# Helkafen/find-tfbs

Hardware: AMD Instinct MI355X
Metric: haplotype-windows scored/sec (higher is better)
Workload: dtype fp4xfp6->f32 bound + int32 exact

## Files before the change

find-tfbs_amd/__init__.py:

```python
import contextlib
import ctypes as C
from collections import namedtuple

from . import _capi
from ._capi import TfbsError, check, lib, tfbs_pattern_desc

TFBS_OK = 0
TFBS_E_NODEVICE = -10
KIND_PWM, KIND_OTHER, KIND_DIPWM = 0, 1, 2
DIR_P, DIR_N = 0, 1
NUCLEOTIDES = "ACGTN"

HIT_DTYPE = [("region", "<u4"), ("haplotype", "<u4"), ("pattern", "<u4"), ("window", "<u4"), ("start", "<u8"),
             ("end", "<u8"), ("score", "<i4"), ("reserved", "<u4")]
HITS_MODES = {"all": 0, "diff": 1}
HITS_HEADER = "#chrom\tregion\thaplotype\tcarriers\tkind\tname\tpattern_id\tstrand\tstart\tend\tscore\tcarrier_ids\n"
BEST_DTYPE = [("region", "<u4"), ("haplotype", "<u4"), ("pattern", "<u4"), ("range", "<u4"), ("window", "<u4"),
              ("n_windows", "<u4"), ("score", "<i4"), ("reserved", "<u4"), ("start", "<u8"), ("end", "<u8")]
BEST_MODES = {"all": 0, "diff": 1}
BEST_HEADER = ("#chrom\tregion\tbed\tinner_start\tinner_end\tname\tpattern_id\thaplotype\tcarriers\tkind\tstrand\t"
               "start\tend\tscore\tdelta\tcarrier_ids\n")
AFFINITY_DTYPE = [("region", "<u4"), ("haplotype", "<u4"), ("pattern", "<u4"), ("range", "<u4"), ("n_windows", "<u4"),
                  ("n_nonzero", "<u4"), ("sum", "<u8")]
AFFINITY_MODES = {"all": 0, "diff": 1}
# ... 254 lines not shown
    return [NUCLEOTIDES.index(n.nuc if isinstance(n, NucleotidePos) else n[0]) for n in hap]


def patch_haplotype(rng, diffs, ref_haplotype):
    L = lib()
    nd = len(diffs)
    dref = [NUCLEOTIDES.index(c) for d in diffs for c in d.reference]
    dalt = [NUCLEOTIDES.index(c) for d in diffs for c in d.alternative]
    n = len(ref_haplotype)
    cap = n + sum(len(d.alternative) for d in diffs) + 8
    on = (C.c_uint8 * cap)()
    op = (C.c_uint64 * cap)()
    nout = C.c_size_t()
    check(L.tfbs_patch_haplotype(
        rng[0], rng[1], nd, (C.c_uint64 * max(1, nd))(*[d.pos for d in diffs]),
        (C.c_uint8 * max(1, len(dref)))(*dref), (C.c_uint32 * max(1, nd))(*[len(d.reference) for d in diffs]),
        (C.c_uint8 * max(1, len(dalt)))(*dalt), (C.c_uint32 * max(1, nd))(*[len(d.alternative) for d in diffs]),
        (C.c_uint8 * max(1, n))(*_nuc_codes(ref_haplotype)),
        (C.c_uint64 * max(1, n))(*[x[1] for x in ref_haplotype]), n, on, op, cap, C.byref(nout)))
    return [NucleotidePos(NUCLEOTIDES[on[i]], op[i]) for i in range(nout.value)]


def counts_as_genotypes(v1, v2, verbose=False):
    n = len(v1)
    maf = C.c_uint32()
    info = C.create_string_buffer(64 + 16 * n)
    gts = C.create_string_buffer(64 + 24 * n)
    r = check(lib().tfbs_counts_as_genotypes((C.c_uint32 * max(1, n))(*v1), (C.c_uint32 * max(1, n))(*v2), n,
                                             C.byref(maf), info, len(info), gts, len(gts)))
    if r != 1:
        return None
    s = info.value.decode()
    counts_part, freqs_part = s.split(";")
    counts = [int(x) for x in counts_part[len("COUNTS="):].split(",")]
    f0, f1, f2 = (int(x) for x in freqs_part[len("freqs="):].split("/"))
    return counts, maf.value, f0, f1, f2, gts.value.decode()


def scores_as_genotypes(left, right, min_spread=1):
    n = len(left)
    maf = C.c_uint32()
    info = C.create_string_buffer(128)
    gts = C.create_string_buffer(16 + 11 * n)
    r = check(lib().tfbs_scores_as_genotypes((C.c_int32 * max(1, n))(*left), (C.c_int32 * max(1, n))(*right), n,
                                             min_spread, C.byref(maf), info, len(info), gts, len(gts)))
    if r != 1:
        return None
    return maf.value, info.value.decode(), gts.value.decode()


PATH_BITS = {"FAST": 1 << 0, "BIG": 1 << 1, "WALK": 1 << 2, "STEPBITS": 1 << 3, "DIRTY_LISTED": 1 << 4,
             "COR_ARENA": 1 << 5, "LISTS_SLICED": 1 << 6, "RUNS_L2": 1 << 7, "HAP_GLOBAL": 1 << 8, "U32": 1 << 9,
             "CNT_ARENA": 1 << 10, "TICKET": 1 << 11, "GIVEUP": 1 << 12, "ASM": 1 << 16, "ASM_HAPS": 1 << 17,
             "ASM_RUNS": 1 << 18, "ASM_HITS": 1 << 19, "ASM_REFS": 1 << 20, "ASM_SCRATCH": 1 << 21}
PATH_WHY_SHIFT = 13


def path_why(word):
    return (word >> PATH_WHY_SHIFT) & 7


class Scanner:

    def __init__(self, patterns, device=0):
        self.patterns = patterns if isinstance(patterns, PatternSet) else PatternSet.from_patterns(patterns)
        self.h = C.c_void_p()
        check(lib().tfbs_ctx_create(device, self.patterns.h, C.byref(self.h)))

    def close(self):
        if getattr(self, "h", None):
            lib().tfbs_ctx_destroy(self.h)
            self.h = None

    def __del__(self):
        self.close()

    def rows_bgzf_blocks(self):
        out = (C.c_uint64 * 3)()
        check(lib().tfbs_ctx_rows_bgzf_blocks(self.h, out))
        return dict(zip(("blocks", "wave", "stored"), (int(x) for x in out)))

    def assembly_trace(self, on=True):
        check(lib().tfbs_ctx_assembly_trace(self.h, 1 if on else 0))

    def assembly_figures(self):
        out = (C.c_uint64 * 8)()
        check(lib().tfbs_ctx_assembly_figures(self.h, out))
        return dict(zip(("left", "arena", "spill", "wide", "leftover", "reruns", "reruns_wide", "reruns_leftover"),
                        (int(x) for x in out)))

    def post_figures(self):
        out = (C.c_uint64 * 4)()
        check(lib().tfbs_ctx_post_figures(self.h, out))
        return dict(zip(("left_out", "reruns_post", "fused", "cand"), (int(x) for x in out)))

    def matches_all(self, haplotype):
        n = len(haplotype)
        nucs = (C.c_uint8 * max(1, n))(*_nuc_codes(haplotype))
        pos = (C.c_uint64 * max(1, n))(*[x[1] for x in haplotype])
        npat = len(self.patterns)
        counts = (C.c_uint32 * max(1, npat))()
        total = C.c_size_t()
        cap = 64
        while True:
            s = (C.c_uint64 * cap)()
            e = (C.c_uint64 * cap)()
            rc = lib().tfbs_matches(self.h, nucs, pos, n, counts, s, e, cap, C.byref(total))
            if rc == -1 and total.value > cap:
                cap = total.value
                continue
            check(rc)
            break
        out, k = [], 0
        for i in range(npat):
            out.append([(s[k + j], e[k + j]) for j in range(counts[i])])
            k += counts[i]
        return out

    def matches(self, pattern_index, haplotype, haplotype_ids=()):
        p = self.patterns[pattern_index]
        ids = tuple(haplotype_ids)
        return [Match(Range(a, b), p.pattern_id, ids) for a, b in self.matches_all(haplotype)[pattern_index]]

    def last_scan_ms(self):
        return lib().tfbs_ctx_last_scan_ms(self.h)

    def last_best_ms(self):
        out = (C.c_double * 2)()
        check(lib().tfbs_ctx_last_best_ms(self.h, out))
        return out[0], out[1]

    def last_affinity_ms(self):
        out = (C.c_double * 2)()
        check(lib().tfbs_ctx_last_affinity_ms(self.h, out))
        return out[0], out[1]

    def last_scores_ms(self):
        out = (C.c_double * 4)()
        check(lib().tfbs_ctx_last_scores_ms(self.h, out))
        return tuple(out)

    def last_effects_ms(self):
        out = (C.c_double * 3)()
        check(lib().tfbs_ctx_last_effects_ms(self.h, out))
        return out[0], out[1], out[2]

    def last_mutscan_ms(self):
        out = (C.c_double * 4)()
        check(lib().tfbs_ctx_last_mutscan_ms(self.h, out))
        return tuple(out)


def mutscan_ring_max_length():
    return lib().tfbs_mutscan_ring_max_length()


def mutscan_kinds_mask(kinds):
    if isinstance(kinds, int):
        return kinds
    names = kinds.split(",") if isinstance(kinds, str) else list(kinds)
    mask = 0
    for k in names:
        mask |= 1 << MUT_KINDS.index(k)
    return mask


# ... 758 lines not shown
```

find-tfbs_amd/_capi.py:

```python
import ctypes as C
import os

HERE = os.path.dirname(os.path.abspath(__file__))
LIB_PATH = os.environ.get("TFBS_LIB") or os.path.join(HERE, "lib", "libtfbs_amd.so")

u8p = C.POINTER(C.c_uint8)
u16p = C.POINTER(C.c_uint16)
u32p = C.POINTER(C.c_uint32)
u64p = C.POINTER(C.c_uint64)
i32p = C.POINTER(C.c_int32)
vp = C.c_void_p


class tfbs_pattern_desc(C.Structure):
    _fields_ = [
        ("pattern_id", C.c_uint16),
        ("direction", C.c_uint8),
        ("kind", C.c_uint8),
        ("length", C.c_uint32),
        ("weights", i32p),
        ("min_score", C.c_int32),
        ("name", C.c_char_p),
    ]

# ... 77 lines not shown
class tfbs_run_ext_affinity(C.Structure):
    _fields_ = tfbs_run_ext_mutscan._fields_ + [("affinity_output", C.c_char_p), ("affinity_mode", C.c_int)]


SIGNATURES = [
    ("tfbs_strerror", C.c_char_p, [C.c_int]),
    ("tfbs_last_error", C.c_char_p, []),
    ("tfbs_version", C.c_char_p, []),
    ("tfbs_patterns_create", C.c_int, [C.POINTER(tfbs_pattern_desc), C.c_size_t, C.POINTER(vp)]),
    ("tfbs_patterns_from_files", C.c_int, [C.c_char_p, C.c_char_p, C.c_float, C.c_char_p, C.c_int, C.POINTER(vp)]),
    ("tfbs_patterns_from_files_di", C.c_int, [C.c_char_p, C.c_char_p, C.c_char_p, C.c_float, C.c_char_p, C.c_int,
                                              C.POINTER(vp)]),
    ("tfbs_patterns_count", C.c_size_t, [vp]),
    ("tfbs_patterns_get", C.c_int, [vp, C.c_size_t, C.POINTER(tfbs_pattern_desc)]),
    ("tfbs_patterns_name_of", C.c_char_p, [vp, C.c_uint16]),
    ("tfbs_patterns_max_length", C.c_uint32, [vp]),
    ("tfbs_patterns_destroy", None, [vp]),
    ("tfbs_patterns_plan_stats", C.c_int, [vp, C.c_uint32, C.c_int, C.POINTER(tfbs_plan_stats)]),
    ("tfbs_patterns_dinuc_stats", C.c_int, [vp, u32p, u32p, u64p]),
    ("tfbs_patterns_dinuc_lut_scores", C.c_int, [vp, C.c_size_t, u8p, C.c_size_t, i32p]),
    ("tfbs_patterns_mfma_bound", C.c_int, [vp, C.c_size_t, C.POINTER(C.c_uint8), C.POINTER(tfbs_mfma_bound)]),
    ("tfbs_patterns_mfma_plan", C.c_int, [vp, C.c_uint32, u8p, C.c_size_t, C.POINTER(C.c_size_t),
                                          C.POINTER(tfbs_mfma_super), C.c_size_t, C.POINTER(C.c_size_t), i32p,
                                          C.c_size_t, C.POINTER(C.c_size_t)]),
    ("tfbs_patterns_score_tails", C.c_int, [vp, C.c_int, C.c_size_t, i32p, C.c_size_t, u64p, u64p]),
    ("tfbs_patterns_pvalue_thresholds", C.c_int, [vp, C.c_int, C.c_double, i32p]),
    ("tfbs_patterns_with_min_scores", C.c_int, [vp, i32p, C.POINTER(vp)]),
    ("tfbs_patterns_from_files_pvalue", C.c_int, [C.c_char_p, C.c_char_p, C.c_char_p, C.c_int, C.c_int, C.c_double,
                                                  C.POINTER(vp)]),
    ("tfbs_pvalue_tile_widths", None, [u32p]),
    ("tfbs_parse_weight", C.c_int, [C.c_char_p, i32p]),
    ("tfbs_parse_threshold_file", C.c_int, [C.c_char_p, C.c_float, i32p]),
    ("tfbs_device_count", C.c_int, [C.POINTER(C.c_int)]),
    ("tfbs_ctx_create", C.c_int, [C.c_int, vp, C.POINTER(vp)]),
    ("tfbs_ctx_destroy", None, [vp]),
    ("tfbs_ctx_sync", C.c_int, [vp]),
    ("tfbs_ctx_set_host_threads", C.c_int, [vp, C.c_uint32]),
    ("tfbs_ctx_last_scan_ms", C.c_float, [vp]),
    ("tfbs_ctx_last_scan_launches", C.c_int, [vp]),
    ("tfbs_ctx_last_mfma_ms", C.c_float, [vp]),
    ("tfbs_ctx_window_lists", C.c_int, [vp, C.POINTER(C.c_uint64), C.POINTER(C.c_double)]),
    ("tfbs_ctx_scan_counters", C.c_int, [vp, C.POINTER(C.c_uint64)]),
    ("tfbs_matches", C.c_int, [vp, u8p, u64p, C.c_size_t, u32p, u64p, u64p, C.c_size_t, C.POINTER(C.c_size_t)]),
    ("tfbs_patch_haplotype", C.c_int, [C.c_uint64, C.c_uint64, C.c_size_t, u64p, u8p, u32p, u8p, u32p, u8p, u64p,
                                       C.c_size_t, u8p, u64p, C.c_size_t, C.POINTER(C.c_size_t)]),
    ("tfbs_batch_create", C.c_int, [vp, C.c_uint32, C.c_int, C.POINTER(vp)]),
    ("tfbs_batch_destroy", None, [vp]),
    ("tfbs_batch_add_bed", C.c_int, [vp, C.c_char_p]),
    ("tfbs_batch_set_window_lmax", C.c_int, [vp, C.c_uint32]),
    ("tfbs_batch_set_build_device", C.c_int, [vp, C.c_int]),
    ("tfbs_batch_hold", C.c_int, [vp, C.c_int]),
    ("tfbs_batch_group_calls", C.c_int, [vp, u64p]),
    ("tfbs_batch_build_stats", C.c_int, [vp, u64p, u64p]),
    ("tfbs_grouper_create", C.c_int, [C.c_int, C.POINTER(vp)]),
    ("tfbs_grouper_destroy", None, [vp]),
    ("tfbs_grouper_group", C.c_int, [vp, C.c_uint32, C.c_size_t, u32p, u32p, u32p, u32p, u64p, u32p, C.c_size_t,
                                     C.POINTER(C.c_size_t), u16p]),
    ("tfbs_batch_patch_stats", C.c_int, [vp, u64p]),
    ("tfbs_batch_region_ext", C.c_int, [vp, C.c_uint64, C.c_uint64, u64p, u64p]),
    ("tfbs_batch_region_begin", C.c_int, [vp, C.c_uint64, C.c_uint64, C.c_char_p, C.c_size_t]),
    ("tfbs_batch_region_add_inner", C.c_int, [vp, C.c_uint32, C.c_uint64, C.c_uint64]),
    ("tfbs_batch_region_add_record_gt", C.c_int, [vp, C.c_uint64, C.c_uint32, C.c_char_p, C.c_char_p, i32p]),
    ("tfbs_batch_region_add_record_carriers", C.c_int, [vp, C.c_uint64, C.c_char_p, C.c_char_p, u32p, C.c_size_t]),
    ("tfbs_batch_region_end", C.c_int, [vp]),
    ("tfbs_batch_num_regions", C.c_size_t, [vp]),
    ("tfbs_batch_num_haplotypes", C.c_size_t, [vp]),
    ("tfbs_batch_num_windows", C.c_uint64, [vp]),
    ("tfbs_batch_num_effective_windows", C.c_uint64, [vp]),
    ("tfbs_batch_num_cell_ops", C.c_uint64, [vp]),
    ("tfbs_batch_num_scan_windows", C.c_uint64, [vp]),
    ("tfbs_batch_num_scan_cell_ops", C.c_uint64, [vp]),
    ("tfbs_batch_input_bytes", C.c_uint64, [vp]),
    ("tfbs_batch_output_bytes", C.c_uint64, [vp]),
    ("tfbs_batch_upload", C.c_int, [vp, vp]),
    ("tfbs_scan", C.c_int, [vp, vp]),
    ("tfbs_batch_download", C.c_int, [vp, vp]),
    ("tfbs_batch_reduce", C.c_int, [vp, vp]),
    ("tfbs_batch_assemble", C.c_int, [vp, vp]),
    ("tfbs_batch_assemble_wait", C.c_int, [vp, vp]),
    ("tfbs_step", C.c_int, [vp, vp]),
    ("tfbs_ctx_last_assemble_ms", C.c_float, [vp]),
    ("tfbs_ctx_assembly_trace", C.c_int, [vp, C.c_int]),
    ("tfbs_batch_assembly_paths", C.c_int, [vp, vp, u32p, C.c_uint32]),
    ("tfbs_ctx_assembly_figures", C.c_int, [vp, u64p]),
    ("tfbs_ctx_post_figures", C.c_int, [vp, u64p]),
    ("tfbs_batch_region_layout", C.c_int, [vp, C.c_size_t, u32p]),
    ("tfbs_batch_region_hap_runs", C.c_int, [vp, C.c_size_t, C.c_uint32, C.POINTER(C.c_int), u32p, u32p, u32p,
                                            C.c_uint32]),
    ("tfbs_batch_region_hap_own_runs", C.c_int, [vp, C.c_size_t, C.c_uint32, C.POINTER(C.c_int), u32p, u32p, u32p,
                                                C.c_uint32]),
    ("tfbs_batch_encode",C.c_int, [vp, vp, C.c_size_t, C.c_size_t]),
    ("tfbs_batch_encode_flags", C.c_int, [vp, vp, C.c_size_t, C.c_size_t, C.c_int]),
    ("tfbs_batch_encode_stats", C.c_int, [vp, u64p]),
    ("tfbs_ctx_rows_bgzf_seconds", C.c_int, [vp, C.POINTER(C.c_double)]),
    ("tfbs_ctx_rows_bgzf_blocks", C.c_int, [vp, u64p]),
    ("tfbs_batch_rows_bgzf", C.c_int, [vp, vp, C.c_size_t, C.c_size_t, C.c_char_p, C.c_uint32, u32p, C.c_int,
                                       u64p, u64p, u64p]),
    ("tfbs_batch_region_num_keys", C.c_int, [vp, C.c_size_t, C.POINTER(C.c_size_t)]),
    ("tfbs_batch_region_key", C.c_int, [vp, C.c_size_t, C.c_size_t, u32p, u64p, u64p, u16p, u32p, u32p]),
    ("tfbs_batch_rows", C.c_int, [vp, C.c_char_p, C.c_uint32, u32p, C.POINTER(C.c_void_p), C.POINTER(C.c_size_t)]),
    ("tfbs_batch_region_rows", C.c_int, [vp, C.c_size_t, C.c_char_p, C.c_uint32, u32p, C.POINTER(C.c_void_p),
                                         C.POINTER(C.c_size_t)]),
    ("tfbs_batch_region_digest", C.c_int, [vp, C.c_size_t, u64p]),
    ("tfbs_batch_region_key_digest_sum", C.c_int, [vp, C.c_size_t, u64p]),
    ("tfbs_batch_region_input_digest", C.c_int, [vp, C.c_size_t, u64p]),
    ("tfbs_batch_region_digests", C.c_int, [vp, C.c_size_t, C.c_size_t, C.c_uint32, C.c_uint32, u64p, u64p, u64p]),
    ("tfbs_batch_region_stats", C.c_int, [vp, C.c_size_t, u32p, u32p]),
    ("tfbs_batch_format_rows", C.c_int, [vp, C.c_char_p, C.c_uint32, C.c_uint32, C.c_size_t, C.c_size_t, u64p,
                                         u64p]),
    ("tfbs_batch_prep_seconds", C.c_int, [vp, C.POINTER(C.c_double)]),
    ("tfbs_batch_hits", C.c_int, [vp, vp, C.c_size_t, C.c_size_t, C.POINTER(C.c_void_p), C.POINTER(C.c_size_t)]),
    ("tfbs_batch_hits_count", C.c_int, [vp, vp, C.c_size_t, C.c_size_t, u64p]),
    ("tfbs_ctx_last_hits_ms", C.c_int, [vp, C.POINTER(C.c_double)]),
    ("tfbs_batch_region_haplotype", C.c_int, [vp, C.c_size_t, C.c_uint32, u8p, u64p, C.c_size_t,
                                              C.POINTER(C.c_size_t), u32p]),
    ("tfbs_batch_region_membership", C.c_int, [vp, C.c_size_t, u32p]),
    ("tfbs_batch_hits_tsv", C.c_int, [vp, C.c_void_p, C.c_size_t, C.c_char_p, C.c_int, C.POINTER(C.c_void_p),
                                      C.POINTER(C.c_size_t)]),
    ("tfbs_batch_best", C.c_int, [vp, vp, C.c_size_t, C.c_size_t, C.POINTER(C.c_void_p), C.POINTER(C.c_size_t)]),
    ("tfbs_batch_region_num_ranges", C.c_int, [vp, C.c_size_t, C.POINTER(C.c_size_t)]),
    ("tfbs_batch_region_range", C.c_int, [vp, C.c_size_t, C.c_size_t, u64p, u64p]),
    ("tfbs_ctx_last_best_ms", C.c_int, [vp, C.POINTER(C.c_double)]),
    ("tfbs_batch_best_tsv", C.c_int, [vp, C.c_void_p, C.c_size_t, C.c_char_p, C.c_int, C.POINTER(C.c_void_p),
                                      C.POINTER(C.c_size_t)]),
    ("tfbs_affinity_weight", C.c_uint64, [C.c_uint64]),
    ("tfbs_patterns_affinity_tops", C.c_int, [vp, i32p]),
    ("tfbs_batch_affinity", C.c_int, [vp, vp, C.c_size_t, C.c_size_t, C.POINTER(C.c_void_p), C.POINTER(C.c_size_t)]),
    ("tfbs_ctx_last_affinity_ms", C.c_int, [vp, C.POINTER(C.c_double)]),
    ("tfbs_batch_affinity_tsv", C.c_int, [vp, C.c_void_p, C.c_size_t, C.c_char_p, C.c_int, C.POINTER(C.c_void_p),
                                          C.POINTER(C.c_size_t)]),
    ("tfbs_batch_keep_variants", C.c_int, [vp, C.c_int]),
    ("tfbs_batch_region_variant", C.c_int, [vp, C.c_size_t, C.c_size_t, u64p, u8p, u8p, C.c_size_t,
                                            C.POINTER(C.c_size_t), C.POINTER(C.c_size_t), u32p, u32p, u32p]),
    ("tfbs_batch_effects", C.c_int, [vp, vp, C.c_size_t, C.c_size_t, C.POINTER(C.c_void_p), C.POINTER(C.c_size_t)]),
    ("tfbs_ctx_last_effects_ms", C.c_int, [vp, C.POINTER(C.c_double)]),
    ("tfbs_batch_effects_tsv", C.c_int, [vp, C.c_void_p, C.c_size_t, C.c_char_p, C.c_int, C.POINTER(C.c_void_p),
                                         C.POINTER(C.c_size_t)]),
    ("tfbs_batch_mutscan", C.c_int, [vp, vp, C.c_size_t, C.c_size_t, C.c_uint32, C.POINTER(C.c_void_p),
                                     C.POINTER(C.c_size_t)]),
    ("tfbs_batch_mutscan_count", C.c_int, [vp, vp, C.c_size_t, C.c_size_t, C.c_uint32, u64p]),
    ("tfbs_mutscan_ring_max_length", C.c_uint32, []),
    ("tfbs_ctx_last_mutscan_ms", C.c_int, [vp, C.POINTER(C.c_double)]),
    ("tfbs_batch_mutscan_tsv", C.c_int, [vp, C.c_void_p, C.c_size_t, C.c_char_p, C.POINTER(C.c_void_p),
                                         C.POINTER(C.c_size_t)]),
    ("tfbs_scores_as_genotypes", C.c_int, [i32p, i32p, C.c_size_t, C.c_uint64, u32p, C.c_char_p, C.c_size_t,
                                           C.c_char_p, C.c_size_t]),
    ("tfbs_batch_score_rows", C.c_int, [vp, vp, C.c_size_t, C.c_size_t, C.c_char_p, C.c_uint32, C.c_uint64, u32p,
                                        C.POINTER(C.c_void_p), C.POINTER(C.c_size_t), u64p]),
    ("tfbs_ctx_last_scores_ms", C.c_int, [vp, C.POINTER(C.c_double)]),
    ("tfbs_free", None, [C.c_void_p]),
    ("tfbs_counts_as_genotypes", C.c_int, [u32p, u32p, C.c_size_t, u32p, C.c_char_p, C.c_size_t, C.c_char_p,
                                           C.c_size_t]),
    ("tfbs_run", C.c_int, [C.c_void_p]),
    ("tfbs_run_ex", C.c_int, [C.c_void_p, C.c_void_p]),
    ("tfbs_bcf_open", C.c_int, [C.c_char_p, C.POINTER(vp)]),
    ("tfbs_inflate_raw", C.c_int, [C.c_void_p, C.c_size_t, C.c_void_p, C.c_size_t]),
    ("tfbs_bcf_close", None, [vp]),
    ("tfbs_bcf_select", C.c_int, [vp, C.POINTER(C.c_size_t), C.c_size_t]),
    ("tfbs_bcf_num_samples", C.c_size_t, [vp]),
    ("tfbs_bcf_indexed", C.c_int, [vp]),
    ("tfbs_bcf_sample_name", C.c_char_p, [vp, C.c_size_t]),
    ("tfbs_bcf_fetch", C.c_int, [vp, C.c_char_p, C.c_uint64, C.c_uint64, C.POINTER(C.c_size_t)]),
    ("tfbs_bcf_set_carriers_mode", C.c_int, [vp, C.c_int]),
    ("tfbs_bcf_record_carriers", C.c_int, [vp, C.c_size_t, C.POINTER(u32p), C.POINTER(C.c_size_t), C.POINTER(C.c_int)]),
    ("tfbs_bcf_record", C.c_int, [vp, C.c_size_t, u64p, u32p, u32p, C.POINTER(C.c_char_p), C.POINTER(C.c_char_p),
                                  C.POINTER(i32p)]),
# ... 47 lines not shown
```

find-tfbs_amd/csrc/ctx.hpp:

```cpp
#pragma once

#include <hip/hip_runtime.h>

#include <algorithm>
#include <atomic>
#include <cerrno>
#include <chrono>
#include <condition_variable>
#include <cstdint>
#include <cstdio>
#include <cstdlib>
#include <cstring>
#include <deque>
#include <functional>
#include <memory>
#include <mutex>
#include <string>
#include <thread>
#include <vector>

#include "batch.hpp"
#include "bgzf_gpu.hpp"
#include "hip_util.hpp"
#include "hits.hpp"
#include "keys.hpp"
#include "patterns.hpp"
#include "rows.hpp"
#include "scan.hpp"
#include "scores.hpp"
#include "tfbs_internal.hpp"

namespace tfbs {

int env_int(const char *name, int dflt);

struct PlanTables {
    DevBuf<DevUnit> fast_units;
    DevBuf<DevPattern> gen_pats;
    DevBuf<DevTile> fast_tiles, gen_tiles;
    DevBuf<int32_t> lut, wfull, gen_w, m_image, m_weights, m_meta;
    DevBuf<DevUnit> di_units;
    DevBuf<DevTile> di_tiles;
    DevBuf<int32_t> di_lut, di_w;
    DevBuf<uint8_t> slot_mfma;
    DevBuf<DevMSuper> m_supers;
    template <class F>
    void each_buf(F &&f) const {
        f(fast_units), f(gen_pats), f(fast_tiles), f(gen_tiles), f(lut), f(wfull), f(gen_w), f(m_image);
        f(m_weights), f(m_meta), f(di_units), f(di_tiles), f(di_lut), f(di_w), f(slot_mfma), f(m_supers);
    }
};

struct Knobs {
    uint32_t tile_blocks = (uint32_t)std::min(36, std::max(8, env_int("TFBS_TILE_BLOCKS", 20)));
    uint32_t haps_per_block = (uint32_t)std::max(8, env_int("TFBS_HAPS_PER_BLOCK", 128));
    bool mfma = env_int("TFBS_MFMA", 1) != 0;
    uint32_t mfma_lds = (uint32_t)std::min(144, std::max(8, env_int("TFBS_MFMA_LDS_KB", 44))) * 1024u;
    uint32_t mfma_hpb = (uint32_t)std::min((int)kMMaxHapsPerBlock, std::max(4, env_int("TFBS_MFMA_HAPS_PER_BLOCK", 64)));
    uint32_t cand_cap = (uint32_t)std::min(1 << 16, std::max(64, env_int("TFBS_CAND_CAP", 1024)));
    uint32_t scan_unit_env = [](int u) { return u == 1 || u == 2 || u == 4 ? u : 0; }(env_int("TFBS_SCAN_UNIT", 0));
    uint32_t scan_unit_words_env = [](const char *uw) {
        return uw && !strcmp(uw, "lds") ? 1u : uw && !strcmp(uw, "global") ? 2u : 0u;
    }(getenv("TFBS_SCAN_UNIT_WORDS"));
    bool debug_over = env_int("TFBS_DEBUG_OVER", 0) != 0;
    bool kf_prof_on = env_int("TFBS_KF_PROF", 0) != 0;
    bool kf_persistent = env_int("TFBS_KF_PERSIST", 1) != 0;
    uint32_t kf_grid = (uint32_t)std::max(0, env_int("TFBS_KF_GRID", 0));
    int kf_big_u = env_int("TFBS_KF_BIGU", (int)key_fast_big_u());
    uint32_t key_fast_max_u = (uint32_t)std::max(0, env_int("TFBS_KEY_FAST_MAXU", 1 << 30));
    uint32_t key_cor_lds = (uint32_t)std::max(0, env_int("TFBS_KEY_COR_LDS", 1 << 30));
    int asm_lean_mode = env_int("TFBS_ASM_LEAN", 1);
    bool post_fuse_env = env_int("TFBS_POST_FUSE", 0) != 0;
    bool step_graphs = env_int("TFBS_STEP_GRAPH", 1) != 0 && !getenv("TFBS_SCAN_PROF") && !kf_prof_on && !debug_over;
};

struct BatchImage {
    DevBuf<uint32_t> words, nmask, counts;
    bool counts_live = false;
    DevBuf<int32_t> posrel, inner;
    DevBuf<DevHap> haps;
    DevBuf<uint32_t> druns;
    DevBuf<DevRegion> regions;
    uint32_t n_regions = 0;
    const tfbs_batch *resident = nullptr;
    uint64_t upload_gen = 0;
    uint32_t mfma_group_words = 0;
    template <class F>
    void each_buf(F &&f) const {
        f(words), f(nmask), f(counts), f(posrel), f(inner), f(haps), f(druns), f(regions);
    }
};

struct WindowLists {
    DevBuf<uint64_t> wl_off[2], wl_tmp;
    DevBuf<uint32_t> wl[2];
    DevBuf<uint16_t> wl16[2];
    DevBuf<uint8_t> gnarrow;
    DevBuf<uint32_t> gorder;
    DevBuf<uint32_t> gcost;
    bool wl_any_narrow = false, wl_any_wide = false;
    DevBuf<uint4> hd, hd2;
    uint64_t wl_entries[2] = {0, 0};
    double wl_seconds = 0;
    uint32_t wl_n_haps = 0;
    uint32_t scan_unit = 1;
    bool wl_share = false;
    DevBuf<uint64_t> sh_off[2], sh_stat;
    DevBuf<uint2> sh[2];
    DevBuf<uint32_t> sh_cur;
    DevBuf<ClassTab> sh_tab;
    uint64_t sh_entries[2] = {0, 0};
    uint64_t sh_listed[2][2] = {{0, 0}, {0, 0}};
    template <class F>
    void each_buf(F &&f) const {
        f(gnarrow), f(gorder), f(hd), f(hd2);
        for (int c = 0; c < 2; c++) f(wl_off[c]), f(wl[c]), f(wl16[c]), f(sh_off[c]), f(sh[c]);
    }
};

struct ScanState {
    Event ev0, ev1;
    Event evk0, evk1;
    Event over_ev;
    bool kernel_timed = false;
    float last_kernel_ms = 0.f, last_ms = 0.f;
    int last_launches = 0;
    bool timing_pending = false;
    bool scanned = false;
    DevBuf<uint32_t> cands;
    DevBuf<uint32_t> hitl, hitn;
    DevBuf<uint32_t> candn;
    DevBuf<uint32_t> ref_hits, ref_count;
    DevBuf<uint32_t> spill, over;
    uint32_t spill_cap = 1u << 16;
    DevBuf<uint32_t> spill_sorted, spill_bcnt, spill_boff;
    bool spill_cnt_ctr = false;
    DevBuf<uint32_t> cand_over;
    uint32_t cand_over_cap = 1u << 20;
    DevBuf<unsigned long long> hits;
    PinnedArray<uint32_t> over_host;
    bool over_pending = false;
    bool over_copied = false;
    bool post_done = false;
    ScanArgs last_margs{};
    uint32_t scan_cand_cap = 1024;
    uint32_t scan_hit_cap = 1024;
    bool post_fuse_ok = false, post_fused = false;
    DevBuf<unsigned long long> scan_prof;
    template <class F>
    void each_buf(F &&f) const {
        f(cands), f(hitl), f(hitn), f(candn), f(ref_hits), f(ref_count), f(spill), f(over), f(spill_sorted);
        f(spill_bcnt), f(spill_boff), f(cand_over), f(hits);
    }
};

struct AsmStages {
    bool wide = true, leftover = true, post = true, post_fused = false;
};

struct AsmState {
    Stream side;
    Event kf_fork, kf_join;
    Event asm_ev, asm_t0, asm_t1;
    DevBuf<uint32_t> asm_scratch;
    DevBuf<uint32_t> key_first, var_counts, asm_redo;
    DevBuf<uint32_t> asm_ctr;
    DevBuf<uint32_t> cor_arena;
    uint32_t cor_cap = 1u << 22;
    DevBuf<uint8_t> key_flags;
    DevBuf<DevVarKey> var_keys;
    uint32_t var_keys_cap = 1u << 16;
    uint64_t var_cap = 1u << 24;
// ... 156 lines not shown
```

find-tfbs_amd/csrc/ctx_assembly.hip:

```cpp
#include "ctx.hpp"

using namespace tfbs;

AsmArgs tfbs::asm_args(tfbs_ctx *ctx, const Batch &B, int mode) {
    AsmArgs a{};
    a.haps = ctx->img.haps.p;
    a.druns = ctx->img.druns.p;
    a.regions = ctx->img.regions.p;
    a.inner = ctx->img.inner.p;
    a.mmeta = ctx->tabs.m_meta.p;
    a.slot_mfma = ctx->tabs.slot_mfma.p;
    a.any_dense = (!ctx->plan.fast_tiles.empty() || !ctx->plan.gen_tiles.empty() || !ctx->plan.di_tiles.empty()) ? 1 : 0;
    a.n_slots = B.n_slots;
    a.hpb = ctx->knobs.mfma_hpb;
    a.hitl = ctx->scan.hitl.p;
    a.hitn = ctx->scan.hitn.p;
    a.cand_cap = ctx->scan.scan_hit_cap;
    a.mfma = ctx->plan.m_supers.empty() ? 0 : 1;
    a.ref_hits = ctx->scan.ref_hits.p;
    a.ref_count = ctx->scan.ref_count.p;
    a.spill_sorted = ctx->scan.spill_sorted.p;
    a.spill_off = ctx->scan.spill_boff.p;
    a.spill_cnt = ctx->scan.spill_cnt_ctr ? ctx->asmb.asm_ctr.p + kAsmCtrWords : ctx->scan.spill_bcnt.p;
    a.spill_count = ctx->plan.m_supers.empty() ? nullptr : ctx->scan.over.p;
    a.spill_cap = ctx->scan.spill_cap;
    a.counts = ctx->img.counts_live ? ctx->img.counts.p : nullptr;
    a.dense_base = ctx->img.counts_live ? 1 : 0;
    a.scratch = ctx->asmb.asm_scratch.p;
    a.mode = mode;
    return a;
}

static int enqueue_assembly(tfbs_ctx *ctx, Batch &B, bool post) {
    int rc;
    const uint64_t n_keys = (uint64_t)(B.inner.size() / 2) * B.n_slots;
    const uint32_t nr = (uint32_t)B.regions.size();
    if ((rc = ctx->asmb.key_first.ensure(std::max<uint64_t>(n_keys, 1))) ||
        (rc = ctx->asmb.key_flags.ensure(std::max<uint64_t>(n_keys, 1))) || (rc = ctx->asmb.asm_ctr.ensure(kAsmCtrWords + asm_bucket_words(nr))) ||
        (rc = ctx->asmb.asm_redo.ensure((size_t)nr + 1)) || (rc = ctx->asmb.cor_arena.ensure(ctx->asmb.cor_cap)))
        return rc;
    if (!ctx->asmb.asm_host) HIP_TRY(ctx->asmb.asm_host.alloc(kAsmCtrWords));
    if (const int vc = env_int("TFBS_VAR_CAP", 0); vc > 0) {
        if (!ctx->asmb.var_cap_forced) {
            ctx->asmb.var_keys_cap = (uint32_t)vc;
            ctx->asmb.var_cap = 4ull * (uint32_t)vc;
            ctx->asmb.var_cap_forced = true;
        }
    } else {
        ctx->asmb.var_keys_cap = std::max<uint32_t>(ctx->asmb.var_keys_cap, (uint32_t)std::min<uint64_t>(n_keys / 16, 1u << 26));
        ctx->asmb.var_cap = std::max<uint64_t>(ctx->asmb.var_cap, std::min<uint64_t>(B.n_counts / 16, 1ull << 28));
    }
    if ((rc = ctx->asmb.var_keys.ensure(ctx->asmb.var_keys_cap)) || (rc = ctx->asmb.var_counts.ensure(ctx->asmb.var_cap))) return rc;
    if (!ctx->step.capturing) HIP_TRY(hipEventRecord(ctx->asmb.asm_t0, ctx->stream));
    const bool mfma = !ctx->plan.m_supers.empty();
    if (!(mfma && post && ctx->asmb.asm_ctr_zeroed && ctx->img.n_regions == nr))
        HIP_TRY(hipMemsetAsync(ctx->asmb.asm_ctr.p, 0, (kAsmCtrWords + (mfma && post ? asm_bucket_words(nr) : 0)) * 4,
                               ctx->stream));
    ctx->asmb.asm_ctr_zeroed = false;
    const bool lean = mfma && post && !ctx->asmb.asm_full && ctx->knobs.asm_lean_mode != 0;
    ctx->asmb.stages.wide = !(lean && (ctx->knobs.asm_lean_mode == 2 || ctx->asmb.prev_spill <= kPostSerial));
    ctx->asmb.stages.leftover = !(lean && (ctx->knobs.asm_lean_mode == 2 || ctx->asmb.prev_redo == 0));
    if (mfma && post) {
        ctx->asmb.stages.post = true;
        ctx->asmb.stages.post_fused = ctx->scan.post_fused;
        if (ctx->scan.post_fused) {
            ctx->asmb.stages.wide = false;
        } else if (asm_skips_post(ctx)) {
            ctx->asmb.stages.post = ctx->asmb.stages.wide = false;
        } else if ((rc = launch_post_fused(ctx->scan.last_margs, !ctx->scan.post_done, ctx->asmb.asm_ctr.p + kCtrWgDone,
                                           std::max<uint32_t>(1, nr), ctx->asmb.asm_ctr.p + kAsmCtrWords, ctx->scan.spill_boff.p,
                                           ctx->scan.spill_sorted.p, ctx->stream, ctx->asmb.stages.wide, ctx->asmb.asm_ctr.p,
                                           ctx->asmb.asm_ctr.p + kCtrNeedWide, lean && ctx->asmb.prev_cand == 0 ? 1u : 256u))) {
            return rc;
        }
        if (ctx->asmb.stages.post) {
            ctx->scan.post_done = true;
            ctx->scan.spill_cnt_ctr = true;
        }
    }
    ctx->scan.post_fused = false;
    AsmArgs a = asm_args(ctx, B, 0);
    if (mfma && !ctx->asmb.stages.post) a.spill_count = nullptr;
    a.report_fast = mfma && !ctx->asmb.stages.post ? 1u : 0u;
    a.key_first = ctx->asmb.key_first.p;
    a.key_flags = ctx->asmb.key_flags.p;
    a.var_keys = ctx->asmb.var_keys.p;
    a.var_keys_cap = ctx->asmb.var_keys_cap;
    a.var_counts = ctx->asmb.var_counts.p;
    a.var_cap = ctx->asmb.var_cap;
    a.var_tot = reinterpret_cast<unsigned long long *>(ctx->asmb.asm_ctr.p + kCtrVarTot);
    a.redo = ctx->asmb.asm_redo.p;
    a.redo_n = ctx->asmb.asm_ctr.p + kCtrRedoN;
    a.fast_max_u = ctx->knobs.key_fast_max_u;
    a.cor_arena = ctx->asmb.cor_arena.p;
    a.cor_cap = ctx->asmb.cor_cap;
    a.cor_used = ctx->asmb.asm_ctr.p + kCtrCorUsed;
    a.cor_lds = ctx->knobs.key_cor_lds;
    a.why = ctx->knobs.debug_over ? ctx->asmb.asm_ctr.p + kCtrWhy : nullptr;
    a.report_src = mfma ? ctx->scan.over.p : nullptr;
    a.report = ctx->asmb.asm_ctr.p;
    a.order = ctx->asmb.asm_order_n == nr ? ctx->asmb.asm_order.p : nullptr;
    a.persist = ctx->knobs.kf_persistent ? 1u : 0u;
    a.next = ctx->asmb.asm_ctr.p + kCtrNext;
    a.grid_cap = ctx->knobs.kf_grid;
    ctx->asmb.asm_traced = ctx->asmb.asm_trace;
    if (ctx->asmb.asm_trace && nr) {
        if ((rc = ctx->asmb.asm_path.ensure(nr))) return rc;
        HIP_TRY(hipMemsetAsync(ctx->asmb.asm_path.p, 0, (size_t)nr * 4, ctx->stream));
        a.path = ctx->asmb.asm_path.p;
    }
    if (ctx->knobs.kf_prof_on && nr) {
        if ((rc = ctx->asmb.kf_prof.ensure((size_t)nr * 16))) return rc;
        HIP_TRY(hipMemsetAsync(ctx->asmb.kf_prof.p, 0, (size_t)nr * 128, ctx->stream));
        a.prof = ctx->asmb.kf_prof.p;
    }
    if ((rc = launch_key_fast(a, nr, a.order ? ctx->asmb.asm_order_big : 0, ctx->stream, ctx->asmb.side, ctx->asmb.kf_fork,
                              ctx->asmb.kf_join, ctx->asmb.stages.leftover)) ||
        (nr == 0 && (rc = launch_asm_report(a.report_src, ctx->asmb.asm_ctr.p, ctx->stream))))
        return rc;
    if (!ctx->step.capturing) HIP_TRY(hipEventRecord(ctx->asmb.asm_t1, ctx->stream));
    HIP_TRY(hipMemcpyAsync(ctx->asmb.asm_host.p, ctx->asmb.asm_ctr.p, 4 * kAsmCtrWords, hipMemcpyDeviceToHost, ctx->stream));
    if (!ctx->step.capturing) HIP_TRY(hipEventRecord(ctx->asmb.asm_ev, ctx->stream));
    ctx->scan.over_pending = false;
    ctx->asmb.asm_batch = &B;
    ctx->asmb.asm_state = 1;
    ctx->asmb.asm_timed = true;
    return TFBS_OK;
}

static int kf_prof_report(tfbs_ctx *ctx, uint32_t nr) {
    std::vector<uint64_t> h((size_t)nr * 16);
    HIP_TRY(hipMemcpy(h.data(), ctx->asmb.kf_prof.p, h.size() * 8, hipMemcpyDeviceToHost));
    double ph[6] = {0, 0, 0, 0, 0, 0}, sz[8] = {0, 0, 0, 0, 0, 0, 0, 0}, mx = 0, at = 0;
    uint32_t n = 0;
    for (uint32_t r = 0; r < nr; r++) {
        const uint64_t *p = &h[(size_t)r * 16];
        if (!p[6]) continue;
        n++;
        for (int k = 0; k < 6; k++) ph[k] += (double)(p[k + 1] - p[k]);
        mx = std::max(mx, (double)(p[6] - p[0]));
        at += (double)p[7];
        for (int k = 0; k < 8; k++) sz[k] += (double)p[8 + k];
    }
    std::vector<std::pair<double, uint32_t>> tot;
    for (uint32_t r = 0; r < nr; r++)
        if (h[(size_t)r * 16 + 6]) tot.push_back({(double)(h[(size_t)r * 16 + 6] - h[(size_t)r * 16]), r});
    std::sort(tot.begin(), tot.end());
    if (!tot.empty()) {
        auto pct = [&](double f) { return tot[std::min(tot.size() - 1, (size_t)(f * tot.size()))].first; };
        fprintf(stderr, "[kf prof] total ticks p50 %.0f p90 %.0f p99 %.0f max %.0f; slowest regions (ticks U rows chunks "
                        "corrections refs):", pct(0.5), pct(0.9), pct(0.99), tot.back().first);
        for (size_t i = tot.size(); i-- > 0 && i + 6 > tot.size();) {
            const uint64_t *p = &h[(size_t)tot[i].second * 16];
            fprintf(stderr, " [%.0f %llu %llu %llu %llu %llu]", tot[i].first, (unsigned long long)p[8],
                    (unsigned long long)p[12], (unsigned long long)p[13], (unsigned long long)p[11],
                    (unsigned long long)p[15]);
        }
        fprintf(stderr, "\n");
    }
    uint64_t t_lo = UINT64_MAX, t_hi = 0;
    double busy = 0;
    for (uint32_t r = 0; r < nr; r++) {
        const uint64_t *p = &h[(size_t)r * 16];
        if (!p[6]) continue;
        t_lo = std::min(t_lo, p[0]);
        t_hi = std::max(t_hi, p[6]);
        busy += (double)(p[6] - p[0]);
    }
    {
        std::vector<std::pair<std::pair<uint64_t, uint64_t>, uint32_t>> ev;
        for (uint32_t r = 0; r < nr; r++)
            if (h[(size_t)r * 16 + 6]) ev.push_back({{h[(size_t)r * 16 + 14], h[(size_t)r * 16]}, r});
        std::sort(ev.begin(), ev.end());
        double gap = 0, late = 0, early_end = 0;
        uint32_t n_gap = 0, n_groups = 0;
        for (size_t i = 0; i < ev.size(); i++) {
            const uint64_t *p = &h[(size_t)ev[i].second * 16];
            const bool first = i == 0 || ev[i - 1].first.first != ev[i].first.first;
            const bool last = i + 1 == ev.size() || ev[i + 1].first.first != ev[i].first.first;
            if (first) {
                n_groups++;
                late += (double)(p[0] - t_lo);
            } else {
                gap += (double)(p[0] - h[(size_t)ev[i - 1].second * 16 + 6]);
                n_gap++;
            }
            if (last) early_end += (double)(t_hi - p[6]);
        }
        if (n_groups)
            fprintf(stderr, "[kf prof] %u workgroups: mean gap between a workgroup's regions %.1f us (%u gaps), first "
                            "region start after the kernel's first %.1f us, last end before the kernel's last %.1f us\n",
                    n_groups, n_gap ? gap / n_gap / 100.0 : 0.0, n_gap, late / n_groups / 100.0, early_end / n_groups / 100.0);
    }
    uint32_t early = 0;
    for (uint32_t r = 0; r < nr; r++)
        if (h[(size_t)r * 16 + 6] && h[(size_t)r * 16] < t_lo + 1000) early++;
    if (t_hi > t_lo)
        fprintf(stderr, "[kf prof] span %.1f us (first region start to last end, 100 MHz ticks), region-time %.1f us: "
                        "%.0f regions in flight on average; %u regions started in the first 10 us\n",
                (t_hi - t_lo) / 100.0, busy / 100.0, busy / (double)(t_hi - t_lo), early);
    const double d = n ? n : 1;
    fprintf(stderr,
            "[kf prof] regions %u of %u ticks/region: descr+hitn %.0f refs %.0f dirty %.0f lists %.0f keys %.0f "
            "chunks %.0f (of which var-list atomics %.0f) (max total %.0f); per region: U %.1f entries %.1f dirty-refs %.1f corrections %.1f rows "
            "%.1f chunks %.2f in-LDS %.2f refs %.1f\n",
            n, nr, ph[0] / d, ph[1] / d, ph[2] / d, ph[3] / d, ph[4] / d, ph[5] / d, at / d, mx, sz[0] / d, sz[1] / d,
            sz[2] / d, sz[3] / d, sz[4] / d, sz[5] / d, sz[6] / d, sz[7] / d);
    return TFBS_OK;
}

int tfbs::assembly_wait(tfbs_ctx *ctx, Batch &B) {
    for (int round = 0; ctx->asmb.asm_state == 1; round++) {
        if (round == 8) return tfbs::fail(TFBS_E_NOMEM, "scan / key lists still full after 8 reruns");
        HIP_TRY(hipEventSynchronize(ctx->asmb.asm_ev));
        const uint32_t nspill = ctx->asmb.asm_host[kCtrOver], ncand = ctx->asmb.asm_host[kCtrOver + 1];
        const uint64_t *vt = reinterpret_cast<const uint64_t *>(ctx->asmb.asm_host.p + kCtrVarTot);
        const uint64_t nk = vt[0], nc = vt[1];
        if (ctx->knobs.debug_over && ctx->asmb.asm_host[kCtrRedoN]) {
            std::vector<uint32_t> redo(ctx->asmb.asm_host[kCtrRedoN]);
            HIP_TRY(hipMemcpy(redo.data(), ctx->asmb.asm_redo.p, redo.size() * 4, hipMemcpyDeviceToHost));
            uint64_t su = 0, sr = 0;
            uint32_t mu = 0, mi = 0;
            for (uint32_t r : redo) {
                const DevRegion &rg = B.regions[r];
                su += rg.hap_count;
                mu = std::max(mu, rg.hap_count);
                mi = std::max(mi, rg.n_inner);
                for (uint32_t l = 0; l < rg.hap_count; l++) sr += B.haps[rg.hap_begin + l].n_druns;
            }
            const uint32_t *why = ctx->asmb.asm_host.p + kCtrWhy;
            fprintf(stderr, "tfbs assembly: %zu regions left to key_asm: mean haplotypes %.1f (max %u), max inner %u, "
                            "mean diff runs %.1f; reasons: shape %u lists %u runs %u refs %u arena(cor) %u arena(cnt) %u\n",
                    redo.size(), (double)su / redo.size(), mu, mi, (double)sr / redo.size(), why[0], why[1], why[2],
                    why[3], why[4], why[5]);
        }
        if (ctx->knobs.debug_over)
            fprintf(stderr, "tfbs assembly: spill %u/%u candidates %u/%u left to key_asm %u arena %u/%u varying keys "
                            "%llu/%u counts %llu/%llu\n", nspill, ctx->scan.spill_cap, ncand, ctx->scan.cand_over_cap,
                    ctx->asmb.asm_host[kCtrRedoN], ctx->asmb.asm_host[kCtrCorUsed], ctx->asmb.cor_cap,
                    (unsigned long long)nk, ctx->asmb.var_keys_cap, (unsigned long long)nc,
                    (unsigned long long)ctx->asmb.var_cap);
        int rc;
        const bool need_post = !ctx->asmb.stages.post && (nspill || ncand);
        const bool need_wide = !ctx->asmb.stages.wide && ctx->asmb.asm_host[kCtrNeedWide], need_left = !ctx->asmb.stages.leftover && ctx->asmb.asm_host[kCtrRedoN];
        if (need_post || need_wide || need_left) {
            ctx->asmb.asm_full = true;
            ctx->asmb.asm_reruns++;
            ctx->asmb.asm_reruns_post += need_post ? 1 : 0;
            ctx->asmb.asm_post_rerun = need_post;
            ctx->asmb.asm_reruns_wide += need_wide ? 1 : 0;
            ctx->asmb.asm_reruns_left += need_left ? 1 : 0;
            rc = enqueue_assembly(ctx, B, true);
            ctx->asmb.asm_full = false;
            if (rc) return rc;
            continue;
        }
        if (ctx->asmb.asm_host[kCtrCorUsed] > ctx->asmb.cor_cap)
            ctx->asmb.cor_cap = (uint32_t)std::min<uint64_t>((uint64_t)ctx->asmb.asm_host[kCtrCorUsed] * 5 / 4, 1u << 30);
        if (nspill > ctx->scan.spill_cap || ncand > ctx->scan.cand_over_cap) {
            grow_cap(ctx->scan.spill_cap, ncand > ctx->scan.cand_over_cap ? 2 * std::max(nspill, 1024u) : nspill, UINT32_MAX / 4);
            grow_cap(ctx->scan.cand_over_cap, ncand, UINT32_MAX / 4);
            const int n = launch_scan(ctx, (uint32_t)B.haps.size(), nullptr, 0);
            if (n < 0) return n;
            if ((rc = enqueue_assembly(ctx, B, true))) return rc;
            continue;
        }
        if (nk > ctx->asmb.var_keys_cap || nc > ctx->asmb.var_cap) {
            if (nk >= (1ull << 32) || nc >= (1ull << 40)) return tfbs::fail(TFBS_E_NOMEM, "too many varying counts");
            ctx->asmb.var_keys_cap = (uint32_t)std::max<uint64_t>(ctx->asmb.var_keys_cap, std::min<uint64_t>(nk + nk / 4 + 1024, UINT32_MAX));
            ctx->asmb.var_cap = std::max<uint64_t>(ctx->asmb.var_cap, nc + nc / 4 + 4096);
            if ((rc = enqueue_assembly(ctx, B, false))) return rc;
            continue;
        }
        ctx->asmb.asm_state = 2;
        ctx->asmb.asm_reruns_wide += ctx->asmb.asm_post_rerun && nspill > kPostSerial ? 1 : 0;
        ctx->asmb.asm_post_rerun = false;
        ctx->asmb.prev_spill = nspill;
        ctx->asmb.prev_redo = ctx->asmb.asm_host[kCtrRedoN];
        ctx->asmb.prev_cand = ncand;
        if (ctx->knobs.kf_prof_on && (rc = kf_prof_report(ctx, (uint32_t)B.regions.size()))) return rc;
    }
    return TFBS_OK;
}

// ... 276 lines not shown
```

find-tfbs_amd/csrc/ctx_scan.hip:

```cpp
#include "ctx.hpp"

using namespace tfbs;

__global__ void zero3_kernel(uint32_t *__restrict__ a, uint32_t na, uint32_t *__restrict__ b, uint32_t nb,
                             uint32_t *__restrict__ c, uint32_t nc) {
    const uint32_t s = gridDim.x * blockDim.x;
    for (uint32_t k = blockIdx.x * blockDim.x + threadIdx.x; k < na || k < nb || k < nc; k += s) {
        if (k < na) a[k] = 0;
        if (k < nb) b[k] = 0;
        if (k < nc) c[k] = 0;
    }
}

constexpr uint32_t kUnitPairs = 2 * kMBlockWaves;
static uint32_t scan_unit_for(const tfbs_ctx *ctx, uint32_t n_groups) {
    if (ctx->knobs.scan_unit_env) return ctx->knobs.scan_unit_env;
    for (int c = 0; c < 2; c++)
        if (ctx->lists.wl_entries[c] > (uint64_t)kUnitPairs * 64 * n_groups) return 1;
    for (uint32_t G = kMMaxUnit; G > 1; G /= 2)
        if (2 * (uint64_t)((n_groups + G - 1) / G) >= 3 * (uint64_t)(2 * ctx->n_cus)) return G;
    return 1;
}

int tfbs::build_lists(tfbs_ctx *ctx, uint32_t n_haps, const std::vector<uint8_t> &narrow, Batch *B) {
    const Plan &P = ctx->plan;
    ctx->lists.wl_share = false;
    ctx->lists.wl_n_haps = n_haps;
    for (int c = 0; c < 2; c++) ctx->lists.sh_entries[c] = ctx->lists.sh_listed[c][0] = ctx->lists.sh_listed[c][1] = 0;
    if (B) B->lists_counted = false;
    if (P.m_supers.empty()) return TFBS_OK;
    const auto t0 = std::chrono::steady_clock::now();
    uint32_t lmin[2] = {0, 0}, span[2] = {0, 0};
    for (const DevMSuper &S : P.m_supers) {
        uint32_t &l = lmin[S.nk > 2 ? 1 : 0];
        l = l ? std::min(l, S.lmin) : S.lmin;
        span[S.nk > 2 ? 1 : 0] = std::max(span[S.nk > 2 ? 1 : 0], S.lmax);
    }
    int rc;
    for (int c = 0; c < 2; c++)
        if (lmin[c] && (rc = ctx->lists.wl_off[c].ensure((size_t)n_haps + 1))) return rc;
    if ((rc = ctx->lists.wl_tmp.ensure(scan_tmp_words((size_t)n_haps + 1))) ||
        (rc = ctx->img.druns.ensure(std::max<size_t>(ctx->img.druns.n, 1))))
        return rc;
    if ((rc = ctx->lists.gnarrow.put(narrow, ctx->stream))) return rc;
    WindowListBufs bufs{};
    for (int c = 0; c < 2; c++) {
        bufs.off[c] = lmin[c] ? ctx->lists.wl_off[c].p : nullptr;
        bufs.list[c] = nullptr;
        bufs.list16[c] = nullptr;
    }
    bufs.gnarrow = narrow.empty() ? nullptr : ctx->lists.gnarrow.p;
    if ((rc = ctx->lists.hd.ensure(std::max<uint32_t>(n_haps, 1))) || (rc = ctx->lists.hd2.ensure(std::max<uint32_t>(n_haps, 1))))
        return rc;
    bufs.hd = ctx->lists.hd.p;
    bufs.hd2 = ctx->lists.hd2.p;
    bufs.scan_tmp = ctx->lists.wl_tmp.p;
    ctx->lists.wl_any_narrow = ctx->lists.wl_any_wide = false;
    for (uint8_t g : narrow) (g ? ctx->lists.wl_any_narrow : ctx->lists.wl_any_wide) = true;
    if (narrow.empty()) ctx->lists.wl_any_wide = true;
    auto ensure = [](void *x, int c, uint64_t n, uint32_t **p, uint16_t **p16) {
        tfbs_ctx *cx = static_cast<tfbs_ctx *>(x);
        if (int e = cx->lists.wl[c].ensure(cx->lists.wl_any_wide ? n : 1)) return e;
        if (int e = cx->lists.wl16[c].ensure(cx->lists.wl_any_narrow ? n : 1)) return e;
        *p = cx->lists.wl[c].p;
        *p16 = cx->lists.wl16[c].p;
        return TFBS_OK;
    };
    const bool share = B && B->dedup && n_haps && env_int("TFBS_SHARE", 1) != 0;
    std::vector<std::pair<uint32_t, uint32_t>> rest;
    if (share) {
        std::vector<ClassTab> tab(2, ClassTab{});
        rest = B->pwm_len_hist;
        for (size_t t = 0; t * kGMetaInts < P.m_meta.size(); t++) {
            const int32_t *gm = &P.m_meta[t * kGMetaInts];
            ClassTab &ct = tab[gm[kGDepth] > 2];
            for (int sn = 0; sn < kMStrands; sn++) {
                if (gm[kGOrig + sn] < 0) continue;
                const uint32_t L = (uint32_t)gm[kGStrandInts * sn + kGLen];
                for (uint32_t r = L; r <= 32; r++) ct.w[r] += 1, ct.c[r] += L;
                for (auto &lc : rest)
                    if (lc.first == L && lc.second) lc.second--;
            }
        }
        if ((rc = ctx->lists.sh_tab.put(tab, ctx->stream)) || (rc = ctx->lists.sh_stat.ensure(4)) ||
            (rc = ctx->lists.sh_cur.ensure(2 * (size_t)n_haps)))
            return rc;
        for (int c = 0; c < 2; c++)
            if (lmin[c] && (rc = ctx->lists.sh_off[c].ensure((size_t)n_haps + 1))) return rc;
        HIP_TRY(hipStreamSynchronize(ctx->stream));
        for (int c = 0; c < 2; c++) bufs.soff[c] = lmin[c] ? ctx->lists.sh_off[c].p : nullptr;
        bufs.scur = ctx->lists.sh_cur.p;
        bufs.stat = ctx->lists.sh_stat.p;
    }
    auto ensure_share = [](void *x, int c, uint64_t n, uint2 **p) {
        tfbs_ctx *cx = static_cast<tfbs_ctx *>(x);
        if (int e = cx->lists.sh[c].ensure(n)) return e;
        *p = cx->lists.sh[c].p;
        return TFBS_OK;
    };
    if ((rc = build_window_lists(ctx->img.haps.p, n_haps, ctx->img.druns.p, lmin, span, ctx->knobs.mfma_hpb, 1, bufs, ctx->lists.wl_entries,
                                 ctx->stream, ensure, ctx, share ? 1u : 0u, ctx->img.regions.p, ctx->img.words.p, ctx->lists.sh_tab.p,
                                 ensure_share, ctx->lists.sh_entries, ctx->lists.sh_listed)))
        return rc;
    ctx->lists.wl_share = share;
    if (share) {
        B->list_windows = ctx->lists.sh_listed[0][0] + ctx->lists.sh_listed[1][0];
        B->list_cell_ops = ctx->lists.sh_listed[0][1] + ctx->lists.sh_listed[1][1];
        for (const auto &lc : rest) {
            if (!lc.second) continue;
            uint64_t nw = 0;
            for (const DevHap &h : B->haps) nw += h.len >= lc.first ? h.len - lc.first + 1 : 0;
            B->list_windows += nw * lc.second;
            B->list_cell_ops += nw * lc.second * lc.first;
        }
        B->lists_counted = true;
    }
    for (int c = 0; c < 2; c++)
        if (!lmin[c]) ctx->lists.wl_off[c].release(), ctx->lists.wl[c].release(), ctx->lists.wl16[c].release();
    ctx->lists.gorder.release();
    ctx->lists.scan_unit = scan_unit_for(ctx, (n_haps + ctx->knobs.mfma_hpb - 1) / ctx->knobs.mfma_hpb);
    if (env_int("TFBS_SCAN_LPT", 1) && n_haps) {
// ... 196 lines not shown
            HIP_TRY(hipEventRecord(ctx->scan.over_ev, ctx->stream));
            ctx->scan.over_copied = true;
        }
        HIP_TRY(hipEventSynchronize(ctx->scan.over_ev));
        uint32_t nspill = ctx->scan.over_host[0];
        const uint32_t ncand = ctx->scan.over_host[1];
        if (ncand > 0 && ncand <= ctx->scan.cand_over_cap && !ctx->scan.post_done) {
            const int f = launch_post_scan(ctx->scan.last_margs, ctx->stream);
            if (f < 0) return f;
            HIP_TRY(hipMemcpyAsync(ctx->scan.over_host.p, ctx->scan.over.p, 8, hipMemcpyDeviceToHost, ctx->stream));
            HIP_TRY(hipStreamSynchronize(ctx->stream));
            nspill = ctx->scan.over_host[0];
        }
        if (ctx->knobs.debug_over) {
            fprintf(stderr, "tfbs_scan overflow lists: spill %u/%u candidates %u/%u\n", nspill, ctx->scan.spill_cap, ncand,
                    ctx->scan.cand_over_cap);
            const size_t nw = ctx->scan.hitn.n;
            std::vector<uint32_t> hn(nw);
            HIP_TRY(hipMemcpy(hn.data(), ctx->scan.hitn.p, nw * 4, hipMemcpyDeviceToHost));
            uint64_t sh = 0, mh = 0;
            for (size_t i = 0; i < nw; i++) sh += hn[i], mh = std::max<uint64_t>(mh, hn[i]);
            fprintf(stderr, "tfbs_scan hit pairs %llu (max per wave %llu) over %zu waves\n", (unsigned long long)sh,
                    (unsigned long long)mh, nw);
        }
        if (nspill <= ctx->scan.spill_cap && ncand <= ctx->scan.cand_over_cap) {
            ctx->scan.over_pending = false;
            ctx->scan.post_done = true;
            if (nspill) {
                const uint32_t nr = std::max<uint32_t>(1, ctx->img.n_regions);
                const int rc = launch_spill_buckets(ctx->scan.over.p, ctx->scan.spill_cap, ctx->scan.spill.p, nr, ctx->scan.spill_bcnt.p,
                                                    ctx->scan.spill_boff.p, ctx->scan.spill_sorted.p, ctx->stream);
                if (rc) return rc;
                ctx->scan.spill_cnt_ctr = false;
            }
            return TFBS_OK;
        }
        grow_cap(ctx->scan.spill_cap, ncand > ctx->scan.cand_over_cap ? 2 * std::max(nspill, 1024u) : nspill, UINT32_MAX / 4);
        grow_cap(ctx->scan.cand_over_cap, ncand, UINT32_MAX / 4);
        const int n = launch_scan(ctx, n_haps, hits, wpp);
        if (n < 0) return n;
    }
    return TFBS_OK;
}

extern "C" {

int tfbs_ctx_group_pairs(tfbs_ctx *ctx, int cls, uint32_t *pairs, size_t cap, size_t *n_groups) {
    if (!ctx || !n_groups || cls < 0 || cls > 1 || (cap && !pairs)) return tfbs::fail(TFBS_E_ARG, "bad argument");
    const uint32_t n = ctx->lists.wl_n_haps, hpb = ctx->knobs.mfma_hpb;
    *n_groups = ((size_t)n + hpb - 1) / hpb;
    if (*n_groups > cap) return cap ? tfbs::fail(TFBS_E_ARG, "group pairs: the array is too small") : TFBS_OK;
    if (!ctx->lists.wl_off[cls].p) {
        for (size_t g = 0; g < *n_groups; g++) pairs[g] = 0;
        return TFBS_OK;
    }
    HIP_TRY(hipSetDevice(ctx->device));
    std::vector<uint64_t> off((size_t)n + 1);
    HIP_TRY(hipStreamSynchronize(ctx->stream));
    HIP_TRY(hipMemcpy(off.data(), ctx->lists.wl_off[cls].p, off.size() * 8, hipMemcpyDeviceToHost));
    for (size_t g = 0; g < *n_groups; g++) {
        const uint64_t nw = off[std::min<size_t>((g + 1) * hpb, n)] - off[g * hpb];
        pairs[g] = (uint32_t)(((nw + 31) / 32 + 1) / 2);
    }
    return TFBS_OK;
}

int tfbs_ctx_share_entries(tfbs_ctx *ctx, int cls, uint32_t *entries, size_t cap, size_t *n_haps) {
    if (!ctx || !n_haps || cls < 0 || cls > 1 || (cap && !entries)) return tfbs::fail(TFBS_E_ARG, "bad argument");
    const uint32_t n = ctx->lists.wl_n_haps;
    *n_haps = n;
    if (n > cap) return cap ? tfbs::fail(TFBS_E_ARG, "share entries: the array is too small") : TFBS_OK;
    if (!ctx->lists.wl_share || !ctx->lists.wl_off[cls].p || !ctx->lists.sh_entries[cls]) {
        for (size_t h = 0; h < n; h++) entries[h] = 0;
        return TFBS_OK;
    }
    HIP_TRY(hipSetDevice(ctx->device));
    std::vector<uint64_t> off((size_t)n + 1);
    HIP_TRY(hipStreamSynchronize(ctx->stream));
    HIP_TRY(hipMemcpy(off.data(), ctx->lists.sh_off[cls].p, off.size() * 8, hipMemcpyDeviceToHost));
    for (size_t h = 0; h < n; h++) entries[h] = (uint32_t)(off[h + 1] - off[h]);
    return TFBS_OK;
}

int tfbs_batch_upload(tfbs_ctx *ctx, tfbs_batch *b) {
    if (!ctx || !b) return tfbs::fail(TFBS_E_ARG, "null argument");
    Batch &B = b->b;
    if (B.pats != ctx->pats) return tfbs::fail(TFBS_E_ARG, "batch and ctx use different pattern sets");
    if (B.open) return tfbs::fail(TFBS_E_STATE, "region still open");
    if (B.slot_pid != ctx->plan.slot_pid) return tfbs::fail(TFBS_E_STATE, "batch slot order differs from the ctx plan");
    HIP_TRY(hipSetDevice(ctx->device));
    uint64_t big = 0;
    for (DevRegion &rg : B.regions) {
        rg.big_off = big;
        if (rg.hap_count > key_asm_lds_counters()) big += rg.hap_count;
    }
    const bool dense = !ctx->plan.fast_tiles.empty() || !ctx->plan.gen_tiles.empty() || !ctx->plan.di_tiles.empty();
    int rc;
    if ((rc = ctx->img.words.put(B.words, ctx->stream)) || (rc = ctx->img.nmask.put(B.nmask, ctx->stream)) ||
        (rc = ctx->img.posrel.put(B.posrel, ctx->stream)) || (rc = ctx->img.haps.put(B.haps, ctx->stream)) ||
        (rc = ctx->img.druns.put(B.druns, ctx->stream)) ||
        (rc = ctx->img.regions.put(B.regions, ctx->stream)) || (rc = ctx->img.inner.put(B.inner, ctx->stream)) ||
        (rc = ctx->asmb.asm_scratch.ensure(std::max<uint64_t>(big, 1))) ||
        (dense && (rc = ctx->img.counts.ensure(std::max<uint64_t>(B.n_counts, 1)))))
        return rc;
    std::vector<uint32_t> order(B.regions.size());
    {
        for (uint32_t i = 0; i < order.size(); i++) order[i] = i;
        std::stable_sort(order.begin(), order.end(), [&](uint32_t x, uint32_t y) {
            return B.regions[x].hap_count > B.regions[y].hap_count;
        });
        if ((rc = ctx->asmb.asm_order.put(order, ctx->stream))) return rc;
        ctx->asmb.asm_order_n = (uint32_t)order.size();
        ctx->asmb.asm_order_big = 0;
        const int big_u = ctx->knobs.kf_big_u;
        while (big_u > 0 && ctx->asmb.asm_order_big < order.size() &&
               B.regions[order[ctx->asmb.asm_order_big]].hap_count > (uint32_t)big_u)
            ctx->asmb.asm_order_big++;
    }
    std::vector<uint8_t> narrow((B.haps.size() + ctx->knobs.mfma_hpb - 1) / ctx->knobs.mfma_hpb, 1);
    for (size_t h = 0; h < B.haps.size(); h++)
        if (B.haps[h].len > kWlNarrowLen) narrow[h / ctx->knobs.mfma_hpb] = 0;
    if ((rc = build_lists(ctx, (uint32_t)B.haps.size(), narrow, &B))) return rc;
    HIP_TRY(hipStreamSynchronize(ctx->stream));
    ctx->img.counts_live = dense;
    ctx->img.resident = b;
    ctx->img.upload_gen++;
    ctx->asmb.prev_spill = ctx->asmb.prev_redo = ctx->asmb.prev_cand = UINT32_MAX;
    ctx->img.mfma_group_words = mfma_group_words(B.haps.data(), (uint32_t)B.haps.size(), ctx->knobs.mfma_hpb);
    ctx->img.n_regions = (uint32_t)B.regions.size();
    ctx->scan.over_pending = false;
    ctx->scan.scanned = false;
    ctx->asmb.asm_state = 0;
    return TFBS_OK;
}

int tfbs_scan(tfbs_ctx *ctx, tfbs_batch *b) {
    if (!ctx || !b) return tfbs::fail(TFBS_E_ARG, "null argument");
    if (ctx->img.resident != b) return tfbs::fail(TFBS_E_STATE, "batch not uploaded to this ctx");
    HIP_TRY(hipSetDevice(ctx->device));
    if (!ctx->step.capturing) HIP_TRY(hipEventRecord(ctx->scan.ev0, ctx->stream));
    ctx->scan.kernel_timed = false;
    const int n = launch_scan(ctx, (uint32_t)b->b.haps.size(), nullptr, 0);
    if (n < 0) return n;
    ctx->scan.scanned = true;
    ctx->asmb.asm_state = 0;
    if (!ctx->step.capturing) HIP_TRY(hipEventRecord(ctx->scan.ev1, ctx->stream));
    ctx->scan.last_launches = n;
    ctx->scan.timing_pending = true;
    b->b.counts_valid = b->b.reduced = false;
    b->b.enc_r0 = b->b.enc_r1 = 0;
    return TFBS_OK;
}

int tfbs_batch_download(tfbs_ctx *ctx, tfbs_batch *b) {
    if (!ctx || !b) return tfbs::fail(TFBS_E_ARG, "null argument");
    if (ctx->img.resident != b) return tfbs::fail(TFBS_E_STATE, "batch not resident on this ctx");
    if (!ctx->scan.scanned) return tfbs::fail(TFBS_E_STATE, "batch not scanned (tfbs_scan)");
    HIP_TRY(hipSetDevice(ctx->device));
    Batch &B = b->b;
    int rc;
    if (ctx->asmb.asm_state == 1 && ctx->asmb.asm_batch == &B && (rc = assembly_wait(ctx, B))) return rc;
    if ((rc = check_overflow(ctx, (uint32_t)B.haps.size()))) return rc;
    if (!ctx->img.counts_live) {
        if ((rc = ctx->img.counts.ensure(std::max<uint64_t>(B.n_counts, 1)))) return rc;
    }
    AsmArgs a = asm_args(ctx, B, 1);
// ... 90 lines not shown
```

find-tfbs_amd/csrc/key_kernels.hip:

```cpp
#include <hip/hip_runtime.h>

#include <mutex>

#include <algorithm>
#include <cstdio>
#include <cstdlib>
#include <string>
#include <type_traits>

#include "keys.hpp"

namespace tfbs {
namespace {

constexpr int kAsmBlock = 256;
constexpr uint32_t kAsmWaves = kAsmBlock / 64;
constexpr uint32_t kAsmCounters = 6144;
constexpr uint32_t kAsmHaps = 1024;

constexpr uint32_t kAsmRuns = 2048;
constexpr uint32_t kAsmHits = 2048;
constexpr uint32_t kAsmRefs = 256;
constexpr uint32_t kAsmKeyWords = 2048;
constexpr uint32_t kAsmKeyWin = 32 * kAsmKeyWords;

__device__ __forceinline__ uint2 spill_range(const AsmArgs &A, uint32_t r) {
    if (!A.spill_count || !*A.spill_count) return make_uint2(0, 0);
    const uint32_t c = A.spill_cnt[r];
    if (c == 0) return make_uint2(0, 0);
    const uint32_t o = A.spill_off[r];
    return make_uint2(o, o + c);
}

__device__ __forceinline__ uint32_t ref_overlaps(const AsmArgs &A, const DevRegion &rg, uint32_t L, uint32_t i,
                                                 uint32_t k0, uint32_t nk) {
    const int32_t *inner = A.inner + 2 * (size_t)rg.inner_off;
    uint32_t mask = 0;
    for (uint32_t k = k0; k < k0 + nk; k++) {
        const int32_t s = inner[2 * k], en = inner[2 * k + 1];
        const uint32_t span = (uint32_t)(en - s);
        if ((uint32_t)((int32_t)i - s) <= span || (uint32_t)((int32_t)(i + L) - 1 - s) <= span) mask |= 1u << (k - k0);
    }
    return mask;
}

__device__ __forceinline__ uint4 make_ref(const AsmArgs &A, const DevRegion &rg, uint32_t g, uint32_t i) {
    const int32_t *meta = A.mmeta + (size_t)(g >> 6) * kGMetaInts;
    const uint32_t sn = g & 63u, L = (uint32_t)meta[kGStrandInts * sn + kGLen];
    const uint32_t dk = (uint32_t)meta[kGDepth] - 1;
    const uint32_t key0 = (uint32_t)meta[kGStrandInts * sn + kGSlot] * rg.n_inner;
    return make_uint4(key0, i, L | (dk << 16), ref_overlaps(A, rg, L, i, 0, min(rg.n_inner, 32u)));
}

template <class F>
__device__ __forceinline__ void visit_hits(const AsmArgs &A, uint32_t r, uint32_t hb, uint32_t U, F &&f) {
    const uint32_t lane = threadIdx.x & 63, wave = threadIdx.x >> 6;
    const uint32_t g_lo = hb / A.hpb, g_hi = (hb + U - 1) / A.hpb;
    if (A.mfma)
        for (uint32_t li = g_lo * kMBlockWaves + wave; li < (g_hi + 1) * kMBlockWaves; li += kAsmWaves) {
            const uint32_t n = A.hitn[li];
            const uint2 *lst = reinterpret_cast<const uint2 *>(A.hitl) + (size_t)(li / kMBlockWaves) * A.cand_cap +
                               (size_t)(li % kMBlockWaves) * (A.cand_cap / kMBlockWaves);
            for (uint32_t e = lane; e < n; e += 64) {
                const uint2 h = lst[e];
                if (h.x - hb < U) f(h.x - hb, h.y);
            }
        }
    const uint2 sp = spill_range(A, r);
    for (uint32_t e = sp.x + threadIdx.x; e < sp.y; e += kAsmBlock) {
        const uint32_t *q = A.spill_sorted + 3 * (size_t)e;
        if (!(q[0] >> 31) && q[1] - hb < U) f(q[1] - hb, q[2]);
    }
}

template <class F>
__device__ __forceinline__ void visit_refs(const AsmArgs &A, uint32_t r, const DevRegion &rg, F &&f) {
    const uint32_t nl = min(A.ref_count[r], kRefPerRegion);
    for (uint32_t t = threadIdx.x; t < nl; t += kAsmBlock)
        f(make_ref(A, rg, A.ref_hits[2 * ((size_t)r * kRefPerRegion + t)],
                   A.ref_hits[2 * ((size_t)r * kRefPerRegion + t) + 1]));
    const uint2 sp = spill_range(A, r);
    for (uint32_t e = sp.x + threadIdx.x; e < sp.y; e += kAsmBlock) {
        const uint32_t *q = A.spill_sorted + 3 * (size_t)e;
        if (q[0] >> 31) f(make_ref(A, rg, q[1], q[2]));
    }
}

__global__ __launch_bounds__(kAsmBlock) void key_asm_kernel(AsmArgs A, const uint32_t *list, const uint32_t *list_n) {
    __shared__ uint32_t s_cnt[kAsmCounters];
    __shared__ uint32_t s_rh[kAsmHaps];
    __shared__ uint2 s_run[kAsmRuns];
    __shared__ uint2 s_hit[kAsmHits];
    __shared__ uint4 s_ref[kAsmRefs];
    __shared__ uint32_t s_bits[kAsmKeyWords], s_rbase[kAsmKeyWords];
    __shared__ uint32_t s_scan[kAsmBlock];
    __shared__ uint32_t s_nhit, s_nref, s_nvar, s_nput;
    __shared__ unsigned long long s_vbase, s_obase;
    const uint32_t tid = threadIdx.x, lane = tid & 63, wave = tid >> 6;
    if (list && A.report && blockIdx.x == 0 && tid < 2) A.report[tid] = A.report_src ? A.report_src[tid] : 0u;
    const uint32_t n_it = list ? *list_n : gridDim.x;
    for (uint32_t it = blockIdx.x; it < n_it; it += gridDim.x) {
    const uint32_t r = list ? list[it] : it;
    __syncthreads();
    [&]() {
    const DevRegion rg = A.regions[r];
    const uint32_t U = rg.hap_count, n_inner = rg.n_inner;
    const uint32_t K = A.n_slots * n_inner;
    const uint64_t ko = (uint64_t)rg.inner_off * A.n_slots;
    auto trace = [&](uint32_t pw) {
        if (A.path && tid == 0) A.path[r] = (list ? A.path[r] : 0u) | TFBS_PATH_ASM | pw;
    };
    if (U == 0 || K == 0) {
        trace(0);
        if (A.mode == 0)
            for (uint32_t j = tid; j < K; j += kAsmBlock) {
                A.key_first[ko + j] = 0;
                A.key_flags[ko + j] = 0;
            }
        return;
    }
    const uint32_t hb = rg.hap_begin;
    uint32_t run0 = 0, run1 = 0;
    for (uint32_t l = 0; l < U; l++)
        if (A.haps[hb + l].flags & HAP_DEDUP) {
            run0 = A.haps[hb + l].rrun_off;
            break;
        }
    for (uint32_t l = U; l-- > 0;)
        if (A.haps[hb + l].flags & HAP_DEDUP) {
            run1 = A.haps[hb + l].rrun_off + A.haps[hb + l].n_rruns;
            break;
        }
    const bool lds_haps = U <= kAsmHaps && run1 - run0 <= kAsmRuns;
    if (lds_haps) {
// ... 207 lines not shown
                }
            }
            __syncthreads();
            const uint32_t nvar = s_nvar;
            if (nvar == 0) continue;
            if (tid == 0) {
                s_vbase = atomicAdd(A.var_tot, (unsigned long long)nvar);
                s_obase = atomicAdd(A.var_tot + 1, (unsigned long long)nvar * U);
                s_nput = 0;
            }
            __syncthreads();
            for (uint32_t rr = wave; rr < nrow; rr += kAsmWaves) {
                const uint32_t *col = cnt + rr * U;
                const uint32_t c0 = col[0];
                uint32_t diff = 0;
                for (uint32_t l = lane; l < U; l += 64) diff |= col[l] ^ c0;
                if (__ballot(diff != 0) == 0) continue;
                const uint32_t j = kw0 + key_of_row(t0 + rr);
                uint32_t at = 0;
                if (lane == 0) at = atomicAdd(&s_nput, 1u);
                at = __shfl(at, 0);
                const uint64_t vi = s_vbase + at;
                const uint64_t off = s_obase + (uint64_t)at * U;
                if (vi < A.var_keys_cap && off + U <= A.var_cap) {
                    if (lane == 0) A.var_keys[vi] = DevVarKey{r, j, off};
                    for (uint32_t l = lane; l < U; l += 64) A.var_counts[off + l] = col[l];
                }
            }
        }
    }
    }();
    }
}

#ifndef TFBS_KF_BLOCK
#define TFBS_KF_BLOCK 256
#endif
constexpr uint32_t kFMaxU = 2048;
constexpr uint32_t kFKeyWords = 512;
constexpr uint32_t kFBatch = 8;
constexpr uint32_t kFNone = 0xFFFFFFFFu;
template <int BLOCK, uint32_t HAP_LDS, uint32_t COR, uint32_t REFS, uint32_t CNT, uint32_t ROWS, uint32_t LISTS>
struct KfShape {
    static constexpr int kBlock = BLOCK;
    static constexpr uint32_t kWaves = BLOCK / 64, kHapLds = HAP_LDS, kCor = COR, kRefs = REFS, kCnt = CNT,
                              kRuns = CNT / 2, kRows = ROWS, kLists = LISTS;
    static_assert(kFMaxU % BLOCK == 0 && HAP_LDS % BLOCK == 0 && LISTS <= BLOCK && REFS <= BLOCK,
                  "key_fast_kernel's per-thread shares");
};
constexpr int kFB = TFBS_KF_BLOCK;
#ifdef TFBS_KF_LDS3
using KfSmall = KfShape<kFB, 4 * kFB, 16 * kFB, kFB, 16 * kFB, 2 * kFB, kFB>;
#elif defined(TFBS_KF_LDS6)
using KfSmall = KfShape<kFB, 2 * kFB, 7 * kFB, kFB, 6 * kFB, kFB, kFB / 2>;
#elif defined(TFBS_KF_LDS8)
using KfSmall = KfShape<kFB, kFB, 4 * kFB, kFB / 2, 4 * kFB, kFB / 2, kFB / 2>;
#else
using KfSmall = KfShape<kFB, 2 * kFB, 14 * kFB, kFB, 12 * kFB, kFB, kFB / 2>;
#endif
using KfBig = KfShape<1024, 2048, 8192, 256, 24576, 1024, 256>;
constexpr uint32_t kFBigU = 384;

__device__ __forceinline__ uint32_t cor_entry(uint32_t key, uint32_t l, uint32_t neg) {
    return (key << 12) | (neg << 11) | l;
}
__device__ __forceinline__ uint32_t cor_key(uint32_t c) { return c >> 12; }
__device__ __forceinline__ bool cor_neg(uint32_t c) { return (c >> 11) & 1u; }
__device__ __forceinline__ uint32_t cor_hap(uint32_t c) { return c & 2047u; }

using KfTyped = std::true_type;
using KfAny = std::false_type;
typedef uint32_t kf_u32x2 __attribute__((ext_vector_type(2)));
__device__ __forceinline__ uint32_t ld_global(const uint32_t *p) {
    return *(const __attribute__((address_space(1))) uint32_t *)p;
}
__device__ __forceinline__ uint2 ld_global(const uint2 *p) {
    const kf_u32x2 v = *(const __attribute__((address_space(1))) kf_u32x2 *)p;
    return make_uint2(v.x, v.y);
}
__device__ __forceinline__ void st_global(uint32_t *p, uint32_t v) {
    *(__attribute__((address_space(1))) uint32_t *)p = v;
}

template <class Put>
__device__ __forceinline__ void wave_push(Put &&put, uint32_t *n, uint32_t cap, bool want, uint32_t v) {
    const uint64_t m = __ballot(want);
    if (!m) return;
    const uint32_t lane = threadIdx.x & 63, leader = (uint32_t)__builtin_ctzll(m);
    uint32_t base = 0;
    if (lane == leader) base = atomicAdd(n, (uint32_t)__popcll(m));
    base = (uint32_t)__shfl((int)base, (int)leader);
    if (want) {
        const uint32_t at = base + __builtin_amdgcn_mbcnt_hi((uint32_t)(m >> 32), __builtin_amdgcn_mbcnt_lo((uint32_t)m, 0));
        if (at < cap) put(at, v);
    }
}

template <uint32_t kFWaves>
__device__ __forceinline__ uint32_t block_excl_scan(uint32_t v, uint32_t *s_w, uint32_t &total) {
    const uint32_t lane = threadIdx.x & 63, wave = threadIdx.x >> 6;
    uint32_t x = v;
#pragma unroll
    for (int o = 1; o < 64; o <<= 1) {
        const uint32_t y = (uint32_t)__shfl_up((int)x, o);
        if (lane >= (uint32_t)o) x += y;
    }
    if (lane == 63) s_w[wave] = x;
    __syncthreads();
    uint32_t pre = 0, tot = 0;
#pragma unroll
    for (uint32_t w = 0; w < kFWaves; w++) {
        const uint32_t t = s_w[w];
        pre += w < wave ? t : 0u;
        tot += t;
    }
    __syncthreads();
    total = tot;
    return pre + x - v;
}

#ifndef TFBS_KF_WAVES
#define TFBS_KF_WAVES 1
#endif
template <class C>
__global__ __launch_bounds__(C::kBlock) __attribute__((amdgpu_waves_per_eu(C::kBlock == 1024 ? 1 : TFBS_KF_WAVES)))
void key_fast_kernel(AsmArgs A, uint32_t first, uint32_t count, uint32_t which) {
    constexpr int kFBlock = C::kBlock;
    constexpr uint32_t kFWaves = C::kWaves, kFHapLds = C::kHapLds, kFCor = C::kCor, kFRefs = C::kRefs,
                       kFCnt = C::kCnt, kFRuns = C::kRuns, kFRows = C::kRows, kFLists = C::kLists;
    constexpr uint32_t kPerW = kFKeyWords >= (uint32_t)kFBlock ? kFKeyWords / kFBlock : 1u;
    __shared__ uint32_t s_cor[kFCor];
    __shared__ uint4 s_ref[kFRefs];
    __shared__ uint32_t s_hap[kFHapLds];
    __shared__ uint32_t s_cnt[kFCnt];
    uint2 *const s_run = reinterpret_cast<uint2 *>(s_cnt);
    __shared__ uint32_t s_bits[kFKeyWords], s_rbase[kFKeyWords];
    __shared__ uint32_t s_rkey[kFRows], s_rr[kFRows];
    __shared__ uint32_t s_loff[kFLists + 1], s_lidx[kFLists];
    __shared__ uint32_t s_w[kFWaves];
    __shared__ uint32_t s_ncor, s_nref, s_run0, s_run1, s_nvar, s_arena, s_ndirty, s_lmax;
    __shared__ unsigned long long s_vbase, s_obase;
    const uint32_t tid = threadIdx.x, lane = tid & 63, wave = tid >> 6;
    auto process = [&](const uint32_t r, const uint32_t by_ticket) {
    auto stamp = [&](uint32_t k, uint64_t v) {
        if (A.prof && tid == 0) A.prof[16 * (size_t)r + k] = v;
    };
    stamp(0, wall_clock64());
    const DevRegion rg = A.regions[r];
    const uint32_t U = rg.hap_count, n_inner = rg.n_inner, K = A.n_slots * n_inner;
    const uint64_t ko = (uint64_t)rg.inner_off * A.n_slots;
    uint32_t pw = TFBS_PATH_FAST | (kFBlock == 1024 ? TFBS_PATH_BIG : 0u) | by_ticket;
    auto trace = [&](uint32_t w) {
        if (A.path && tid == 0) A.path[r] = w;
    };
    if (U == 0 || K == 0) {
        trace(pw);
        for (uint32_t j = tid; j < K; j += kFBlock) {
            A.key_first[ko + j] = 0;
            A.key_flags[ko + j] = 0;
        }
        return;
    }
    auto give_up = [&](uint32_t why) {
        if (tid == 0) {
            A.redo[atomicAdd(A.redo_n, 1u)] = r;
            if (A.why) atomicAdd(A.why + why, 1u);
        }
        trace(pw | TFBS_PATH_GIVEUP | (why << TFBS_PATH_WHY_SHIFT));
    };
    if (U > (kFMaxU < A.fast_max_u ? kFMaxU : A.fast_max_u) || K > 32 * kFKeyWords || n_inner > 32) return give_up(0);
    const uint32_t hb = rg.hap_begin;
    const bool refs_on = A.mfma && rg.ref_hap != UINT32_MAX;
    if (tid == 0) {
        s_ncor = s_nref = s_run1 = s_ndirty = s_lmax = 0;
        s_run0 = kFNone;
    }
    __syncthreads();
    constexpr uint32_t kPer = kFMaxU / kFBlock;
    uint32_t roff[kPer], rn[kPer], lmax = 0;
#pragma unroll
    for (uint32_t q = 0; q < kPer; q++) {
        const uint32_t l = tid + q * kFBlock;
        roff[q] = kFNone;
        rn[q] = 0;
        if (l < U) {
            const DevHap &h = A.haps[hb + l];
            lmax = max(lmax, h.len);
            if (h.flags & HAP_DEDUP) {
                roff[q] = h.rrun_off;
                rn[q] = h.n_rruns;
                atomicMin(&s_run0, h.rrun_off);
                atomicMax(&s_run1, h.rrun_off + h.n_rruns);
            }
        }
    }
    const uint32_t g_lo = hb / A.hpb, g_hi = (hb + U - 1) / A.hpb;
    const uint32_t nl = A.mfma ? (g_hi + 1 - g_lo) * kMBlockWaves : 0u;
    auto list_idx = [&](uint32_t t) -> uint32_t { return g_lo * kMBlockWaves + t; };
    uint32_t lcnt = 0, lidx = 0;
    for (uint32_t t = tid; t < nl; t += kFBlock) {
        const uint32_t i = list_idx(t);
        if (t == tid) lidx = i;
        lcnt += A.hitn[i];
    }
    uint32_t n_ent = 0;
    const uint32_t loff = block_excl_scan<kFWaves>(lcnt, s_w, n_ent);
    if (tid == 0 && rg.ref_hap != UINT32_MAX) lmax = max(lmax, A.haps[rg.ref_hap].len);
    if (lmax) atomicMax(&s_lmax, lmax);
    const bool lists_staged = nl <= kFLists;
    if (lists_staged && tid < nl) {
        s_lidx[tid] = lidx;
        s_loff[tid] = loff;
    }
    if (lists_staged && tid == 0) s_loff[nl] = n_ent;
    stamp(1, wall_clock64());
    const uint32_t run0 = s_run0, nruns = s_run0 == kFNone ? 0u : s_run1 - s_run0;
    if (!lists_staged) pw |= TFBS_PATH_LISTS_SLICED;
    if (nruns >= 65536) return give_up(2);
    if (nruns > kFRuns) pw |= TFBS_PATH_RUNS_L2;
#pragma unroll
    for (uint32_t q = 0; q < kFHapLds / kFBlock; q++) {
        const uint32_t l = tid + q * kFBlock;
        if (l < U) s_hap[l] = roff[q] == kFNone ? kFNone : (roff[q] - run0) | (rn[q] << 16);
    }
    auto hap_info = [&](uint32_t l) -> uint32_t {
        if (l < kFHapLds) return s_hap[l];
        const DevHap &h = A.haps[hb + l];
        return (h.flags & HAP_DEDUP) ? (h.rrun_off - run0) | (h.n_rruns << 16) : kFNone;
    };
    const bool runs_lds = nruns <= kFRuns;
    const uint2 *const druns = reinterpret_cast<const uint2 *>(A.druns) + (nruns ? run0 : 0u);
    auto run_at = [&](auto typed, uint32_t k) -> uint2 {
        if constexpr (decltype(typed)::value) {
            return s_run[k];
        } else {
            if (runs_lds) return s_run[k];
            return ld_global(druns + k);
        }
    };
    if (runs_lds)
        for (uint32_t k = tid; k < nruns; k += kFBlock)
            s_run[k] = make_uint2(A.druns[2 * (run0 + k)], A.druns[2 * (run0 + k) + 1]);
    const uint2 sp = spill_range(A, r);
    if (refs_on) {
        const uint32_t n = min(A.ref_count[r], kRefPerRegion);
        if (tid < n) {
            const size_t o = 2 * ((size_t)r * kRefPerRegion + tid);
            const uint32_t at = atomicAdd(&s_nref, 1u);
            if (at < kFRefs) s_ref[at] = make_ref(A, rg, A.ref_hits[o], A.ref_hits[o + 1]);
        }
        for (uint32_t e = sp.x + tid; e < sp.y; e += kFBlock) {
            const uint32_t *q = A.spill_sorted + 3 * (size_t)e;
            if (q[0] >> 31) {
                const uint32_t at = atomicAdd(&s_nref, 1u);
                if (at < kFRefs) s_ref[at] = make_ref(A, rg, q[1], q[2]);
            }
        }
    }
    __syncthreads();
    const uint32_t nref = s_nref;
    if (nref > kFRefs) return give_up(3);
    const bool pairwise = (uint64_t)U * nref <= 65536;
    if (!pairwise) pw |= TFBS_PATH_WALK;
    if (!pairwise) {
        uint4 mine = make_uint4(0, 0, 0, 0);
        uint32_t rank = 0;
        if (tid < nref) {
            mine = s_ref[tid];
            for (uint32_t j = 0; j < nref; j++) {
                const uint32_t w = s_ref[j].y;
                rank += (w < mine.y || (w == mine.y && j < tid)) ? 1u : 0u;
            }
        }
        __syncthreads();
        if (tid < nref) s_ref[rank] = mine;
        __syncthreads();
    }
    stamp(2, wall_clock64());
    auto dirty_masks = [&](auto typed, auto &&f) {
        for (uint32_t l0 = wave * 64; l0 < U; l0 += kFBlock) {
            const uint32_t l = l0 + lane;
            const uint32_t x = l < U ? hap_info(l) : kFNone;
            const uint32_t k0 = x == kFNone ? 0u : x & 0xFFFFu, k1 = x == kFNone ? 0u : k0 + (x >> 16);
            for (uint32_t p0 = 0; p0 < nref; p0 += 64) {
                const uint32_t np = min(64u, nref - p0);
                uint32_t rw = 0, re = 0;
                if (lane < np) {
                    const uint4 q = s_ref[p0 + lane];
                    rw = q.y;
                    re = q.y + (q.z & 0xFFFFu) - 1;
                }
                uint64_t m = 0;
                for (uint32_t i = 0; __ballot(i < k1 - k0) != 0; i++) {
                    uint2 ab = make_uint2(0xFFFFFFFFu, 0u);
                    if (i < k1 - k0) ab = run_at(typed, k0 + i);
                    for (uint32_t p = 0; p < np; p++) {
                        const uint32_t w = (uint32_t)__builtin_amdgcn_readlane((int)rw, (int)p);
                        const uint32_t e = (uint32_t)__builtin_amdgcn_readlane((int)re, (int)p);
                        if (ab.x <= e && ab.y >= w) m |= 1ull << p;
                    }
                }
                f(l, p0, m);
            }
        }
    };
    auto dirty_walk = [&](auto typed, auto &&f) {
        for (uint32_t l = tid; l < U; l += kFBlock) {
            const uint32_t x = hap_info(l);
            if (x == kFNone) continue;
            const uint32_t k0 = x & 0xFFFFu, k1 = k0 + (x >> 16);
            uint32_t p = 0;
            for (uint32_t k = k0; k < k1 && p < nref; k++) {
                const uint2 ab = run_at(typed, k);
                const uint32_t a = ab.x, b = ab.y;
                const uint32_t lo = a >= kMChunkCols * kMMaxChunks - 1 ? a - (kMChunkCols * kMMaxChunks - 1) : 0u;
                while (p < nref && s_ref[p].y < lo) p++;
                for (; p < nref && s_ref[p].y <= b; p++) {
                    const uint4 q = s_ref[p];
                    bool dirty = false;
                    for (uint32_t k2 = k0; k2 < k1 && !dirty; k2++) {
                        const uint2 r2 = run_at(typed, k2);
                        dirty = run_meets(r2.x, r2.y, q.y, q.z & 0xFFFFu);
                    }
                    if (dirty) f(l, q);
                }
            }
        }
    };
    auto slots = [&](uint32_t c, uint32_t *ctr) -> uint32_t {
        if (!__ballot(c > 1)) {
            const uint64_t m = __ballot(c != 0);
            if (!m) return 0;
            const uint32_t leader = (uint32_t)__builtin_ctzll(m);
            uint32_t base = 0;
            if (lane == leader) base = atomicAdd(ctr, (uint32_t)__popcll(m));
            return (uint32_t)__shfl((int)base, (int)leader) +
                   __builtin_amdgcn_mbcnt_hi((uint32_t)(m >> 32), __builtin_amdgcn_mbcnt_lo((uint32_t)m, 0));
        }
        uint32_t x = c;
#pragma unroll
        for (int o = 1; o < 64; o <<= 1) {
            const uint32_t y = (uint32_t)__shfl_up((int)x, o);
            if (lane >= (uint32_t)o) x += y;
// ... 95 lines not shown
                const uint32_t e = e0 + q * kFBlock + tid;
                h[q] = make_uint2(hb + U, 0);
                if (e < tot) {
                    uint32_t lo = 0, hi = nlc - 1;
                    while (lo < hi) {
                        const uint32_t mid = (lo + hi + 1) / 2;
                        if (s_loff[mid] <= e) lo = mid;
                        else hi = mid - 1;
                    }
                    const uint32_t idx = s_lidx[lo];
                    h[q] = hitl[(size_t)(idx / kMBlockWaves) * A.cand_cap +
                                (size_t)(idx % kMBlockWaves) * (A.cand_cap / kMBlockWaves) + (e - s_loff[lo])];
                }
            }
#pragma unroll
            for (uint32_t q = 0; q < kFBatch; q++)
                wave_push(put, &s_ncor, need, h[q].x - hb < U, cor_entry(h[q].y, h[q].x - hb, 0));
        }
        __syncthreads();
    }
    for (uint32_t e0 = sp.x; e0 < sp.y; e0 += kFBlock) {
        const uint32_t e = e0 + tid;
        bool want = false;
        uint32_t v = 0;
        if (e < sp.y) {
            const uint32_t *q = A.spill_sorted + 3 * (size_t)e;
            want = !(q[0] >> 31) && q[1] - hb < U;
            v = cor_entry(q[2], q[1] - hb, 0);
        }
        wave_push(put, &s_ncor, need, want, v);
    }
    if (!dirty_listed && nref) {
        auto put_in = [&](uint32_t at, uint32_t v) {
            if (at < need) cor_st(typed, at, v);
        };
        if (pairwise)
            dirty_masks(typed, [&](uint32_t l, uint32_t p0, uint64_t m) { (void)list_mask(l, p0, m, &s_ncor, put_in); });
        else
            dirty_walk(typed, [&](uint32_t l, const uint4 &q) {
                uint32_t at = atomicAdd(&s_ncor, (uint32_t)__popc(q.w));
                for (uint32_t m = q.w; m; m &= m - 1, at++) put_in(at, cor_entry(q.x + __builtin_ctz(m), l, 1));
            });
    }
    for (uint32_t w = tid; w < nw; w += kFBlock) s_bits[w] = 0;
    __syncthreads();
    stamp(4, wall_clock64());
    nA = s_ncor, nB = in_lds && dirty_listed ? nD : 0u, ncor = nA + nB;
    for (uint32_t e = tid; e < nA; e += kFBlock) {
        const uint32_t c = cor_ld(typed, e);
        if (!cor_neg(c)) atomicOr(&s_bits[cor_key(c) >> 5], 1u << (cor_key(c) & 31u));
    }
    if (tid < nref)
        for (uint32_t m = s_ref[tid].w; m; m &= m - 1) {
            const uint32_t key = s_ref[tid].x + __builtin_ctz(m);
            atomicOr(&s_bits[key >> 5], 1u << (key & 31u));
        }
    if (A.any_dense)
        for (uint32_t j = tid; j < K; j += kFBlock)
            if (!A.slot_mfma[j / n_inner]) atomicOr(&s_bits[j >> 5], 1u << (j & 31u));
    __syncthreads();
    {
        constexpr uint32_t per = kPerW;
        uint32_t mine = 0;
#pragma unroll
        for (uint32_t q = 0; q < per; q++) {
            const uint32_t w = tid * per + q;
            if (w < nw) mine += __popc(s_bits[w]);
        }
        uint32_t run = block_excl_scan<kFWaves>(mine, s_w, T);
#pragma unroll
        for (uint32_t q = 0; q < per; q++) {
            const uint32_t w = tid * per + q;
            if (w < nw) {
                s_rbase[w] = run;
                run += __popc(s_bits[w]);
            }
        }
    }
    };
    if (in_lds && runs_lds) lists_and_rows(KfTyped{});
    else lists_and_rows(KfAny{});
    stamp(5, wall_clock64());
    auto row_of = [&](uint32_t j) { return s_rbase[j >> 5] + __popc(s_bits[j >> 5] & ((1u << (j & 31)) - 1u)); };
    const bool half = 4 * (s_lmax + 64) < 65536 && A.cor_lds != 0;
    uint32_t rows_per = min((half ? 2 : 1) * kFCnt / U, kFRows);
    uint16_t *const cnt16 = reinterpret_cast<uint16_t *>(s_cnt);
    bool h16 = half, cnt_arena = false;
    uint32_t *cnt_g = A.cor_arena;
    if ((T + rows_per - 1) / rows_per > 32 || A.cor_lds == 0) {
        h16 = false;
        cnt_arena = true;
        pw |= TFBS_PATH_CNT_ARENA;
        rows_per = min(T, kFRows);
        if (tid == 0) {
            s_arena = kFNone;
            const uint32_t want = rows_per * U, at = atomicAdd(A.cor_used, want);
            if (at <= A.cor_cap && want <= A.cor_cap - at) s_arena = at;
        }
        __syncthreads();
        if (s_arena == kFNone) return give_up(5);
        cnt_g = A.cor_arena + s_arena;
    }
    pw |= (h16 ? 0u : TFBS_PATH_U32) | (U > kFHapLds ? TFBS_PATH_HAP_GLOBAL : 0u);
    for (uint32_t j = tid; j < K; j += kFBlock)
        if (!((s_bits[j >> 5] >> (j & 31)) & 1u)) {
            A.key_first[ko + j] = 0;
            A.key_flags[ko + j] = 0;
        }
    const uint64_t dense_base = A.dense_base ? A.haps[hb].count_off : 0;
    uint64_t t_atomics = 0;
    auto chunks = [&](auto typed) {
    constexpr bool kTyped = decltype(typed)::value;
    auto cor_top = [&](uint32_t e) -> uint32_t { return kFCor - nB + (e - nA); };
    auto cor_at = [&](uint32_t e) -> uint32_t {
        if constexpr (kTyped) return s_cor[e < nA ? e : cor_top(e)];
        else return e < nA ? cor_ld(typed, e) : s_cor[cor_top(e)];
    };
    auto cnt_set = [&](uint32_t x, uint32_t v) {
        if (kTyped || h16) cnt16[x] = (uint16_t)v;
        else if (cnt_arena) st_global(cnt_g + x, v);
        else s_cnt[x] = v;
    };
    auto cnt_add = [&](uint32_t x, uint32_t d) {
        if (kTyped || h16) atomicAdd(&s_cnt[x >> 1], d << (16 * (x & 1u)));
        else if (cnt_arena) atomicAdd(&cnt_g[x], d);
        else atomicAdd(&s_cnt[x], d);
    };
    auto count_at = [&](uint32_t x) -> uint32_t {
        if (kTyped || h16) return (uint32_t)cnt16[x];
        if (cnt_arena) return ld_global(cnt_g + x);
        return s_cnt[x];
    };
    for (uint32_t e = tid; e < ncor; e += kFBlock) {
        const uint32_t c = cor_at(e), v = (row_of(cor_key(c)) << 12) | (c & 4095u);
        if (e < nA) cor_st(typed, e, v);
        else s_cor[cor_top(e)] = v;
    }
    uint32_t dedup_bits = 0;
    for (uint32_t i = 0, l = lane; l < U; i++, l += 64)
        if (hap_info(l) != kFNone) dedup_bits |= 1u << i;
    for (uint32_t t0 = 0; t0 < T; t0 += rows_per) {
        const uint32_t nrow = min(rows_per, T - t0);
        __syncthreads();
        if (tid == 0) s_nvar = 0;
        {
            constexpr uint32_t per = kPerW;
#pragma unroll
            for (uint32_t q = 0; q < per; q++) {
                const uint32_t w = tid * per + q;
                if (w >= nw) continue;
                uint32_t t = s_rbase[w], b = s_bits[w];
                if (t >= t0 + nrow || t + __popc(b) <= t0) continue;
                for (; b; b &= b - 1, t++)
                    if (t - t0 < nrow) s_rkey[t - t0] = 32 * w + __builtin_ctz(b);
            }
        }
        for (uint32_t rr = tid; rr < nrow; rr += kFBlock) s_rr[rr] = 0;
        __syncthreads();
        if (tid < nref)
            for (uint32_t m = s_ref[tid].w; m; m &= m - 1) {
                const uint32_t t = row_of(s_ref[tid].x + __builtin_ctz(m)) - t0;
                if (t < nrow) atomicAdd(&s_rr[t], 1u);
            }
        __syncthreads();
        for (uint32_t rr = wave; rr < nrow; rr += kFWaves) {
            const uint32_t j = s_rkey[rr], R = s_rr[rr];
            const bool dense = A.any_dense && !A.slot_mfma[j / n_inner];
            for (uint32_t i = 0, l = lane; l < U; i++, l += 64) {
                const uint32_t v = dense ? A.counts[dense_base + (uint64_t)j * rg.count_stride + l]
                                         : ((dedup_bits >> i) & 1u ? R : 0u);
                cnt_set(rr * U + l, v);
            }
        }
        __syncthreads();
        for (uint32_t e = tid; e < ncor; e += kFBlock) {
            const uint32_t c = cor_at(e);
            const uint32_t t = cor_key(c) - t0;
            if (t < nrow) cnt_add(t * U + cor_hap(c), cor_neg(c) ? 0xFFFFFFFFu : 1u);
        }
        __syncthreads();
        for (uint32_t rr = wave; rr < nrow; rr += kFWaves) {
            const uint32_t c0 = count_at(rr * U);
            uint32_t any = 0, diff = 0;
            for (uint32_t l = lane; l < U; l += 64) {
                const uint32_t c = count_at(rr * U + l);
                any |= c;
                diff |= c ^ c0;
            }
            const bool a = __ballot(any != 0) != 0, v = __ballot(diff != 0) != 0;
            if (lane == 0) {
                const uint32_t j = s_rkey[rr];
                A.key_first[ko + j] = c0;
                A.key_flags[ko + j] = (uint8_t)((a ? KEY_ANY : 0) | (v ? KEY_VARIES : 0));
                s_rr[rr] = v ? atomicAdd(&s_nvar, 1u) : kFNone;
            }
        }
        __syncthreads();
        const uint64_t ta = A.prof ? wall_clock64() : 0;
        if (tid == 0 && s_nvar) {
            s_vbase = atomicAdd(A.var_tot, (unsigned long long)s_nvar);
            s_obase = atomicAdd(A.var_tot + 1, (unsigned long long)s_nvar * U);
        }
        __syncthreads();
        if (A.prof) t_atomics += wall_clock64() - ta;
        for (uint32_t rr = wave; rr < nrow; rr += kFWaves) {
            const uint32_t slot = s_rr[rr];
            if (slot == kFNone) continue;
            const uint64_t vi = s_vbase + slot, off = s_obase + (uint64_t)slot * U;
            if (vi >= A.var_keys_cap || off + U > A.var_cap) continue;
            if (lane == 0) A.var_keys[vi] = DevVarKey{r, s_rkey[rr], off};
            for (uint32_t l = lane; l < U; l += 64) A.var_counts[off + l] = count_at(rr * U + l);
        }
    }
    };
    if (in_lds && h16) chunks(KfTyped{});
    else chunks(KfAny{});
    stamp(6, wall_clock64());
    stamp(7, t_atomics);
    stamp(8, U);
    stamp(9, n_ent);
    stamp(10, nD);
    stamp(11, ncor);
    stamp(12, T);
    stamp(13, (T + rows_per - 1) / rows_per);
    stamp(14, blockIdx.x | (which << 24));
    stamp(15, nref);
    trace(pw);
    };
    __shared__ uint32_t s_tk;
    const bool tickets = A.persist && gridDim.x < count;
    uint32_t i = blockIdx.x;
    while (i < count) {
        uint32_t tk = 0;
        if (tickets && tid == 0) tk = gridDim.x + atomicAdd(A.next + which, 1u);
        process(A.order ? A.order[first + i] : first + i, i == blockIdx.x ? 0u : (uint32_t)TFBS_PATH_TICKET);
        if (!tickets) break;
        if (tid == 0) s_tk = tk;
        __syncthreads();
        i = s_tk;
        __syncthreads();
    }
    if (A.report_fast && blockIdx.x == 0 && tid < 2) A.report[tid] = A.report_src ? A.report_src[tid] : 0u;
}

__global__ __launch_bounds__(256) void spill_hist_kernel(const uint32_t *__restrict__ over, uint32_t cap,
                                                          const uint32_t *__restrict__ spill, uint32_t *__restrict__ bcnt) {
    const uint32_t n = min(over[0], cap);
    for (uint32_t e = blockIdx.x * 256 + threadIdx.x; e < n; e += gridDim.x * 256)
        atomicAdd(&bcnt[spill[3 * (size_t)e] & 0x7FFFFFFFu], 1u);
}

__global__ __launch_bounds__(1024) void spill_scan_kernel(const uint32_t *__restrict__ over, uint32_t *__restrict__ bcnt,
                                                          uint32_t n, uint32_t *__restrict__ boff) {
    __shared__ uint32_t s[1024];
    if (over[0] == 0) return;
    uint32_t carry = 0;
    for (uint32_t b0 = 0; b0 < n; b0 += 1024) {
        const uint32_t i = b0 + threadIdx.x;
        const uint32_t v = i < n ? bcnt[i] : 0;
        s[threadIdx.x] = v;
        __syncthreads();
        for (uint32_t o = 1; o < 1024; o <<= 1) {
            const uint32_t t = threadIdx.x >= o ? s[threadIdx.x - o] : 0;
            __syncthreads();
            s[threadIdx.x] += t;
            __syncthreads();
        }
        if (i < n) {
            boff[i] = carry + s[threadIdx.x] - v;
            bcnt[i] = 0;
        }
        carry += s[1023];
        __syncthreads();
    }
    if (threadIdx.x == 0) boff[n] = carry;
}

__global__ __launch_bounds__(256) void spill_scatter_kernel(const uint32_t *__restrict__ over, uint32_t cap,
                                                            const uint32_t *__restrict__ spill,
                                                            const uint32_t *__restrict__ boff,
                                                            uint32_t *__restrict__ bfill, uint32_t *__restrict__ out) {
    const uint32_t n = min(over[0], cap);
    for (uint32_t e = blockIdx.x * 256 + threadIdx.x; e < n; e += gridDim.x * 256) {
        const uint32_t r = spill[3 * (size_t)e] & 0x7FFFFFFFu;
        const uint32_t at = boff[r] + atomicAdd(&bfill[r], 1u);
        out[3 * (size_t)at] = spill[3 * (size_t)e];
        out[3 * (size_t)at + 1] = spill[3 * (size_t)e + 1];
        out[3 * (size_t)at + 2] = spill[3 * (size_t)e + 2];
    }
}

constexpr int kPairBlock = 512;
constexpr uint32_t kPairSlots = 2 * kEncMaxPairs;
constexpr uint32_t kPairEmpty = 0xFFFFFFFFu;

__device__ __forceinline__ uint32_t pair_slot(uint32_t key) { return (key * 0x9E3779B1u) >> (32 - 14); }
static_assert(kPairSlots == 1u << 14, "pair_slot hashes into 2^14 slots");

__global__ __launch_bounds__(kPairBlock) void pair_table_kernel(const uint64_t *__restrict__ rows, uint32_t n_samples,
                                                                uint32_t *__restrict__ pab, uint32_t *__restrict__ pcnt,
                                                                uint32_t *__restrict__ pair_n,
                                                                uint16_t *__restrict__ pidx) {
    __shared__ uint32_t s_key[kPairSlots];
    __shared__ uint32_t s_val[kPairSlots];
    __shared__ uint32_t s_n, s_over, s_pos;
    const uint32_t r = blockIdx.x, tid = threadIdx.x, lane = tid & 63;
    const uint16_t *m = reinterpret_cast<const uint16_t *>(rows[r]);
    if (!m) {
        if (tid == 0) pair_n[r] = kPairEmpty;
        return;
    }
    for (uint32_t t = tid; t < kPairSlots; t += kPairBlock) {
        s_key[t] = kPairEmpty;
        s_val[t] = 0;
    }
    if (tid == 0) {
        s_n = 0;
        s_over = 0;
// ... 369 lines not shown
```

find-tfbs_amd/csrc/keys.hpp:

```cpp
#pragma once

#include <hip/hip_runtime.h>

#include <algorithm>
#include <cstddef>
#include <cstdint>

#include "batch.hpp"
#include "scan.hpp"

namespace tfbs {

struct AsmArgs {
    const DevHap *haps;
    const uint32_t *druns;
    const DevRegion *regions;
    const int32_t *inner;
    const int32_t *mmeta;
    const uint8_t *slot_mfma;
    uint32_t any_dense;
    uint32_t n_slots;
    uint32_t hpb;
    const uint32_t *hitl, *hitn;
    uint32_t cand_cap;
    uint32_t mfma;
    const uint32_t *ref_hits, *ref_count;
    const uint32_t *spill_sorted, *spill_off, *spill_cnt;
    const uint32_t *spill_count;
    uint32_t spill_cap;
    uint32_t *counts;
    uint32_t dense_base;
    uint32_t *scratch;
    int mode;
    uint32_t *key_first;
    uint8_t *key_flags;
    DevVarKey *var_keys;
    uint32_t var_keys_cap;
    uint32_t *var_counts;
    uint64_t var_cap;
    unsigned long long *var_tot;
    uint32_t *redo, *redo_n;
    uint32_t fast_max_u;
    uint32_t *cor_arena;
    uint32_t cor_cap;
    uint32_t *cor_used;
    uint32_t cor_lds;
    uint32_t *why;
    const uint32_t *report_src;
    uint32_t *report;
    uint32_t report_fast;
    const uint32_t *order;
    uint32_t persist;
    uint32_t *next;
    uint64_t *prof;
    uint32_t *path;
    uint32_t grid_cap;
};

enum AsmCtr : uint32_t {
    kCtrOver = 0,
    kCtrRedoN = 2,
    kCtrCorUsed = 3,
    kCtrVarTot = 4,
    kCtrWhy = 8,
    kCtrNext = 16,
    kCtrWgDone = 18,
    kCtrNeedWide = 20,
    kCtrPostDone = 21,
    kAsmCtrWords = 24,
};
inline size_t asm_bucket_words(uint32_t nr) { return 2 * ((size_t)std::max<uint32_t>(1, nr) + 1); }

int launch_key_asm(const AsmArgs &a, uint32_t n_regions, hipStream_t stream);
int launch_key_fast(const AsmArgs &a, uint32_t n_regions, uint32_t n_big, hipStream_t stream, hipStream_t side,
                    hipEvent_t fork, hipEvent_t join, bool leftover = true);
uint32_t key_fast_big_u();
int launch_asm_report(const uint32_t *over, uint32_t *ctr, hipStream_t stream);
uint32_t key_asm_lds_counters();
int launch_spill_buckets(const uint32_t *over, uint32_t cap, const uint32_t *spill, uint32_t n_regions, uint32_t *bcnt,
                         uint32_t *boff, uint32_t *sorted, hipStream_t stream, bool bcnt_zeroed = false);
int launch_pair_table(const uint64_t *rows, uint32_t n_regions, uint32_t n_samples, uint32_t *pab, uint32_t *pcnt,
                      uint32_t *pair_n, uint16_t *pidx, hipStream_t stream);
int launch_memb_fill(const uint32_t *meta, const uint32_t *ids, const uint16_t *loc, uint32_t n_rows, uint32_t Hp,
                     uint16_t *memb, hipStream_t stream);
int launch_key_encode(const uint32_t *var_counts, const DevVarKey *keys, uint32_t n_keys, const uint32_t *pab,
                      const uint32_t *pcnt, const uint32_t *pair_n, const uint16_t *pidx, uint32_t region0,
                      uint32_t n_samples, EncHdr *hdr, uint32_t *vals, uint32_t *hist, uint8_t *codes,
                      hipStream_t stream);
int launch_val_compact(const uint32_t *vals, const uint32_t *hist, uint32_t n_keys, const uint32_t *off, uint32_t *ov,
                       uint32_t *oh, hipStream_t stream);
int launch_code_compact(const uint8_t *codes, uint32_t n_keys, uint32_t n_samples, const uint64_t *off, uint8_t *dst,
                        hipStream_t stream);

}
```

find-tfbs_amd/csrc/scan.hpp:

```cpp
#pragma once

#include <hip/hip_runtime.h>

#include <cstdint>

#include "tfbs_internal.hpp"

namespace tfbs {

struct ScanArgs {
    const DevTile *tiles;
    uint32_t n_tiles;
    const DevUnit *units;
    const DevPattern *gpats;
    const int32_t *lut;
    const int32_t *wfull;
    const int32_t *gw;
    const DevHap *haps;
    uint32_t n_haps;
    uint32_t hap_base;
    const DevRegion *regions;
    const int32_t *inner;
    const uint32_t *words;
    const uint32_t *nmask;
// ... 18 lines not shown
    uint32_t *candn;
    const uint32_t *wlist[2];
    const uint16_t *wlist16[2];
    const uint4 *hd;
    const uint4 *hd2;
    const uint8_t *gnarrow;
    const uint32_t *gorder;
    uint32_t unit;
    uint32_t unit_words, unit_lds, unit_lds_words;
    const uint64_t *wlist_off[2];
    const uint64_t *share_off[2];
    const uint2 *share[2];
    uint32_t dedup;
    const uint32_t *druns;
    uint32_t n_regions;
    uint32_t *ref_hits;
    uint32_t *ref_count;
    uint32_t *spill;
    uint32_t *over;
    uint32_t spill_cap;
    uint32_t *cand_over;
    uint32_t cand_over_cap;
    uint32_t *post_done;
    uint32_t post_regions;
    uint32_t *post_bcnt, *post_boff, *post_sorted, *post_report, *post_need_wide;
    unsigned long long *prof;
};
constexpr uint32_t kScanProfWords = 16;
constexpr uint32_t kRefPerRegion = 64;
constexpr uint32_t kMBlockWaves = 8;
constexpr uint32_t kCandWords = 2;
constexpr uint32_t kMMaxUnit = 4;

struct LaunchConfig {
    int minw = 2;
    size_t lds_bytes = 0;
};

int launch_fast(const ScanArgs &a, const LaunchConfig &cfg, uint32_t n_haps, hipStream_t stream);
int launch_generic(const ScanArgs &a, uint32_t n_haps, hipStream_t stream);
int fast_kernel_set_lds(const LaunchConfig &cfg);
int launch_dinuc(const ScanArgs &a, size_t lds_bytes, uint32_t n_haps, hipStream_t stream);
int dinuc_kernel_set_lds(size_t lds_bytes);
constexpr uint32_t kMWaveCands = 48;
constexpr uint64_t kMLaunchGroups = ((1ull << 31) - 1) / kMMaxUnit * kMMaxUnit;
int launch_mfma_all(const ScanArgs &a, const DevMSuper *supers, uint32_t n_supers, uint32_t group_words, uint32_t n_haps,
                    hipStream_t stream);
int launch_post_scan(const ScanArgs &a, hipStream_t stream);
constexpr uint32_t kPostSerial = 8192;
int launch_post_fused(const ScanArgs &a, bool cand, uint32_t *done, uint32_t n_regions, uint32_t *bcnt, uint32_t *boff,
                      uint32_t *sorted, hipStream_t stream, bool wide = true, uint32_t *report = nullptr,
                      uint32_t *need_wide = nullptr, uint32_t cand_grid = 256);
uint32_t mfma_group_words(const DevHap *haps, uint32_t n_haps, uint32_t hpb);
constexpr uint32_t kMMaxHapsPerBlock = 64;
constexpr uint32_t kWlNarrowLen = 1024;
struct WindowListBufs {
    uint64_t *off[2];
    uint64_t *scan_tmp;
    uint32_t *list[2];
    uint16_t *list16[2];
    const uint8_t *gnarrow;
    uint4 *hd;
    uint4 *hd2;
    uint64_t list_cap[2];
    uint64_t *soff[2];
    uint32_t *scur;
    uint2 *share[2];
    uint64_t *stat;
};
struct ClassTab {
    uint32_t w[33], c[33];
};
size_t scan_tmp_words(size_t n);
int exclusive_scan(uint64_t *x, uint64_t n, uint64_t *tmp, hipStream_t stream);
int group_costs(const uint64_t *off0, const uint64_t *off1, uint32_t n_haps, uint32_t hpb, uint32_t w0, uint32_t w1,
                uint32_t *cost, hipStream_t stream);
int build_window_lists(const DevHap *haps, uint32_t n_haps, const uint32_t *druns, const uint32_t lmin[2],
                       const uint32_t span[2], uint32_t hpb, uint32_t dedup, WindowListBufs &bufs, uint64_t total[2], hipStream_t stream,
                       int (*ensure_list)(void *ctx, int c, uint64_t n, uint32_t **p, uint16_t **p16),
                       void *ensure_ctx, uint32_t share = 0, const DevRegion *regions = nullptr,
                       const uint32_t *words = nullptr, const ClassTab *tab = nullptr,
                       int (*ensure_share)(void *ctx, int c, uint64_t n, uint2 **p) = nullptr,
                       uint64_t shared[2] = nullptr, uint64_t listed[2][2] = nullptr);
size_t mfma_lds_fixed();

}
```

find-tfbs_amd/csrc/window_lists.hip:

```cpp
#include <hip/hip_runtime.h>

#include <algorithm>
#include <string>

#include "scan.hpp"

namespace tfbs {
namespace {

template <class F>
__device__ __forceinline__ uint32_t for_windows(const DevHap &hm, const uint32_t *druns, uint32_t lmin, uint32_t S,
                                                uint32_t dedup, F &&f) {
    if (hm.len < lmin) return 0;
    const uint32_t nw = hm.len - lmin + 1;
    if (!dedup || !(hm.flags & HAP_DEDUP)) {
        f(0u, nw);
        return nw;
    }
    uint32_t n = 0, next = 0;
    for (uint32_t k = 0; k < hm.n_druns; k++) {
        const uint32_t a = druns[2 * (hm.drun_off + k)], b = druns[2 * (hm.drun_off + k) + 1];
        const uint32_t lo = max(next, a >= S - 1 ? a - (S - 1) : 0u), hi = min(b, nw - 1) + 1;
        if (hi > lo) {
            f(lo, hi);
// ... 143 lines not shown
        rw += (uint32_t)__shfl_down((int)rw, o);
        rc += (uint32_t)__shfl_down((int)rc, o);
    }
    if (lane == 0) {
        cnt[h] = own;
        hstat[2 * (size_t)h] = rw;
        hstat[2 * (size_t)h + 1] = rc;
    }
}

__global__ __launch_bounds__(256) void wl_share_fill_kernel(const DevHap *__restrict__ haps, uint32_t n,
                                                            const DevRegion *__restrict__ regions,
                                                            const uint32_t *__restrict__ druns,
                                                            const uint32_t *__restrict__ words, uint32_t lmin, uint32_t S,
                                                            uint32_t hpb, const uint64_t *__restrict__ off,
                                                            uint32_t *__restrict__ list, uint16_t *__restrict__ list16,
                                                            const uint8_t *__restrict__ gnarrow,
                                                            const uint64_t *__restrict__ soff,
                                                            uint32_t *__restrict__ scur, uint2 *__restrict__ share) {
    const uint32_t h = __builtin_amdgcn_readfirstlane(blockIdx.x * 4 + (threadIdx.x >> 6)), lane = threadIdx.x & 63;
    if (h >= n) return;
    const DevHap hm = haps[h];
    uint64_t at = off[h];
    const uint64_t end = off[h + 1];
    const uint32_t hl = h % hpb;
    const bool narrow = gnarrow && gnarrow[h / hpb];
    for_shared_windows(haps, regions, druns, words, h, hm, lmin, S, lane, [&](uint32_t w, bool active, uint32_t d) {
        const bool own = active && d == h;
        const uint64_t ob = __ballot(own);
        const uint64_t q = at + __builtin_amdgcn_mbcnt_hi((uint32_t)(ob >> 32), __builtin_amdgcn_mbcnt_lo((uint32_t)ob, 0));
        if (own && q < end) {
            if (narrow) list16[q] = (uint16_t)((w << 6) | hl);
            else list[q] = (w << 6) | hl;
        }
        at += (uint32_t)__popcll(ob);
        uint32_t len;
        if (sharer_run(active && d != h, d, lane, &len)) {
            const uint64_t e = soff[d] + atomicAdd(scur + d, 1u);
            if (e < soff[d + 1]) share[e] = make_uint2(h, w | ((w + len) << 16));
        }
    });
}

__global__ __launch_bounds__(256) void pair_sum_kernel(const uint32_t *__restrict__ x, uint32_t n,
                                                       unsigned long long *__restrict__ sum) {
    unsigned long long a = 0, b = 0;
    for (uint32_t k = blockIdx.x * 256 + threadIdx.x; k < n; k += gridDim.x * 256) {
        a += x[2 * (size_t)k];
        b += x[2 * (size_t)k + 1];
    }
    for (uint32_t o = 32; o; o >>= 1) {
        a += (unsigned long long)__shfl_down((long long)a, o);
        b += (unsigned long long)__shfl_down((long long)b, o);
    }
    if ((threadIdx.x & 63) == 0 && (a | b)) {
        atomicAdd(sum, a);
        atomicAdd(sum + 1, b);
    }
}

__global__ __launch_bounds__(256) void group_cost_kernel(const uint64_t *__restrict__ off0,
                                                         const uint64_t *__restrict__ off1, uint32_t n_haps, uint32_t hpb,
                                                         uint32_t n_groups, uint32_t w0, uint32_t w1,
                                                         uint32_t *__restrict__ cost) {
    const uint32_t g = blockIdx.x * 256 + threadIdx.x;
    if (g >= n_groups) return;
    const uint32_t h0 = g * hpb, h1 = min(h0 + hpb, n_haps);
    uint64_t c = 0;
    if (off0) c += (off0[h1] - off0[h0] + 2 * kMWindows - 1) / (2 * kMWindows) * w0;
    if (off1) c += (off1[h1] - off1[h0] + 2 * kMWindows - 1) / (2 * kMWindows) * w1;
    cost[g] = (uint32_t)min<uint64_t>(c, 0xFFFFFFFFu);
}

__global__ __launch_bounds__(256) void hd_kernel(const DevHap *__restrict__ haps, uint32_t n, uint4 *__restrict__ hd,
                                                  uint4 *__restrict__ hd2) {
    const uint32_t h = blockIdx.x * 256 + threadIdx.x;
    if (h < n) {
        const DevHap x = haps[h];
        hd[h] = make_uint4(x.word_off, x.len, x.flags, x.nmask_off);
        hd2[h] = make_uint4(x.region, x.pos_off, x.drun_off, x.n_druns);
    }
}

constexpr uint32_t kScanThreads = 1024, kScanTile = 4 * kScanThreads;
__global__ __launch_bounds__(kScanThreads) void scan_tile_kernel(uint64_t *__restrict__ x, uint64_t n,
                                                                 uint64_t *__restrict__ sums) {
    __shared__ uint64_t s[2][kScanThreads];
    const uint32_t t = threadIdx.x;
    const uint64_t base = (uint64_t)blockIdx.x * kScanTile + 4 * t;
    uint64_t v[4], tot = 0;
    for (int k = 0; k < 4; k++) {
        v[k] = base + k < n ? x[base + k] : 0;
        tot += v[k];
    }
    int cur = 0;
    s[0][t] = tot;
    __syncthreads();
    for (uint32_t o = 1; o < kScanThreads; o <<= 1) {
        s[cur ^ 1][t] = s[cur][t] + (t >= o ? s[cur][t - o] : 0);
        cur ^= 1;
        __syncthreads();
    }
    uint64_t run = s[cur][t] - tot;
    for (int k = 0; k < 4; k++) {
        if (base + k < n) x[base + k] = run;
        run += v[k];
    }
    if (t == kScanThreads - 1) sums[blockIdx.x] = s[cur][t];
}

__global__ __launch_bounds__(256) void scan_add_kernel(uint64_t *__restrict__ x, uint64_t n,
                                                       const uint64_t *__restrict__ sums) {
    const uint64_t add = sums[blockIdx.x];
    for (uint32_t k = threadIdx.x; k < kScanTile; k += 256) {
        const uint64_t i = (uint64_t)blockIdx.x * kScanTile + k;
        if (i < n) x[i] += add;
    }
}

}

int exclusive_scan(uint64_t *x, uint64_t n, uint64_t *tmp, hipStream_t stream) {
    const uint64_t nt = (n + kScanTile - 1) / kScanTile;
    if (nt == 0) return TFBS_OK;
    hipLaunchKernelGGL(scan_tile_kernel, dim3((uint32_t)nt), dim3(kScanThreads), 0, stream, x, n, tmp);
    if (nt > 1) {
        if (int rc = exclusive_scan(tmp, nt, tmp + nt, stream)) return rc;
        hipLaunchKernelGGL(scan_add_kernel, dim3((uint32_t)nt), dim3(256), 0, stream, x, n, tmp);
    }
    const hipError_t e = hipGetLastError();
    if (e != hipSuccess) return fail(TFBS_E_HIP, std::string("scan kernels: ") + hipGetErrorString(e));
    return TFBS_OK;
}

uint32_t mfma_group_words(const DevHap *haps, uint32_t n_haps, uint32_t hpb) {
    uint32_t mx = 0;
    for (uint32_t h0 = 0; h0 < n_haps; h0 += hpb) {
        const uint32_t hl = std::min(h0 + hpb, n_haps) - 1;
        mx = std::max(mx, haps[hl].word_off + (haps[hl].len + 15) / 16 + 3 - haps[h0].word_off);
    }
    return mx;
}

size_t scan_tmp_words(size_t n) {
    size_t w = 0;
    for (size_t nt = (n + kScanTile - 1) / kScanTile; nt > 0; nt = nt > 1 ? (nt + kScanTile - 1) / kScanTile : 0) w += nt;
    return w + 1;
}

int build_window_lists(const DevHap *haps, uint32_t n_haps, const uint32_t *druns, const uint32_t lmin[2],
                       const uint32_t span[2], uint32_t hpb, uint32_t dedup, WindowListBufs &bufs, uint64_t total[2], hipStream_t stream,
                       int (*ensure_list)(void *ctx, int c, uint64_t n, uint32_t **p, uint16_t **p16),
                       void *ensure_ctx, uint32_t share, const DevRegion *regions, const uint32_t *words,
                       const ClassTab *tab, int (*ensure_share)(void *ctx, int c, uint64_t n, uint2 **p),
                       uint64_t shared[2], uint64_t listed[2][2]) {
    if (n_haps && bufs.hd) hipLaunchKernelGGL(hd_kernel, dim3((n_haps + 255) / 256), dim3(256), 0, stream, haps, n_haps,
                                             bufs.hd, bufs.hd2);
    share = share && dedup && n_haps;
    if (share) {
        hipError_t e = hipMemsetAsync(bufs.stat, 0, 4 * sizeof(uint64_t), stream);
        if (e != hipSuccess) return fail(TFBS_E_HIP, std::string("window lists: ") + hipGetErrorString(e));
    }
    for (int c = 0; c < 2; c++) {
        total[c] = 0;
        if (shared) shared[c] = 0;
        if (listed) listed[c][0] = listed[c][1] = 0;
        if (!lmin[c]) continue;
        const uint32_t S = span[c] ? span[c] : kMChunkCols * (c ? 4 : 2);
        if (share) {
            unsigned long long *scnt = reinterpret_cast<unsigned long long *>(bufs.soff[c]);
            hipError_t e = hipMemsetAsync(bufs.soff[c], 0, ((size_t)n_haps + 1) * 8, stream);
            if (e == hipSuccess) e = hipMemsetAsync(bufs.scur, 0, (size_t)n_haps * 8, stream);
            if (e != hipSuccess) return fail(TFBS_E_HIP, std::string("window lists: ") + hipGetErrorString(e));
            hipLaunchKernelGGL(wl_share_count_kernel, dim3(n_haps / 4 + 1), dim3(256), 0, stream, haps, n_haps, regions,
                               druns, words, lmin[c], S, tab + c, bufs.off[c], scnt, bufs.scur);
            hipLaunchKernelGGL(pair_sum_kernel, dim3(256), dim3(256), 0, stream, bufs.scur, n_haps,
                               reinterpret_cast<unsigned long long *>(bufs.stat) + 2 * c);
            int rc;
            if ((rc = exclusive_scan(bufs.off[c], (uint64_t)n_haps + 1, bufs.scan_tmp, stream)) ||
                (rc = exclusive_scan(bufs.soff[c], (uint64_t)n_haps + 1, bufs.scan_tmp, stream)))
                return rc;
            uint64_t ns = 0;
            e = hipMemcpyAsync(&total[c], bufs.off[c] + n_haps, 8, hipMemcpyDeviceToHost, stream);
            if (e == hipSuccess) e = hipMemcpyAsync(&ns, bufs.soff[c] + n_haps, 8, hipMemcpyDeviceToHost, stream);
            if (e == hipSuccess) e = hipMemcpyAsync(listed[c], bufs.stat + 2 * c, 16, hipMemcpyDeviceToHost, stream);
            if (e == hipSuccess) e = hipStreamSynchronize(stream);
            if (e != hipSuccess) return fail(TFBS_E_HIP, std::string("window list size: ") + hipGetErrorString(e));
            shared[c] = ns;
            if ((rc = ensure_list(ensure_ctx, c, std::max<uint64_t>(total[c], 1), &bufs.list[c], &bufs.list16[c])) ||
                (rc = ensure_share(ensure_ctx, c, std::max<uint64_t>(ns, 1), &bufs.share[c])))
                return rc;
            e = hipMemsetAsync(bufs.scur, 0, (size_t)n_haps * 4, stream);
            if (e != hipSuccess) return fail(TFBS_E_HIP, std::string("window lists: ") + hipGetErrorString(e));
            hipLaunchKernelGGL(wl_share_fill_kernel, dim3((n_haps + 3) / 4), dim3(256), 0, stream, haps, n_haps, regions,
                               druns, words, lmin[c], S, hpb, bufs.off[c], bufs.list[c], bufs.list16[c], bufs.gnarrow,
                               bufs.soff[c], bufs.scur, bufs.share[c]);
            e = hipGetLastError();
            if (e != hipSuccess) return fail(TFBS_E_HIP, std::string("wl_share_fill_kernel: ") + hipGetErrorString(e));
            continue;
        }
        hipLaunchKernelGGL(wl_count_kernel, dim3(n_haps / 256 + 1), dim3(256), 0, stream, haps, n_haps, druns, lmin[c],
                           S, dedup, bufs.off[c]);
        if (int rc = exclusive_scan(bufs.off[c], (uint64_t)n_haps + 1, bufs.scan_tmp, stream)) return rc;
        hipError_t e = hipMemcpyAsync(&total[c], bufs.off[c] + n_haps, 8, hipMemcpyDeviceToHost, stream);
        if (e == hipSuccess) e = hipStreamSynchronize(stream);
        if (e != hipSuccess) return fail(TFBS_E_HIP, std::string("window list size: ") + hipGetErrorString(e));
        if (int rc = ensure_list(ensure_ctx, c, std::max<uint64_t>(total[c], 1), &bufs.list[c], &bufs.list16[c]))
            return rc;
        if (n_haps)
            hipLaunchKernelGGL(wl_fill_kernel, dim3((n_haps + 3) / 4), dim3(256), 0, stream, haps, n_haps, druns,
                               lmin[c], S, dedup, hpb, bufs.off[c], bufs.list[c], bufs.list16[c], bufs.gnarrow);
        e = hipGetLastError();
        if (e != hipSuccess) return fail(TFBS_E_HIP, std::string("wl_fill_kernel: ") + hipGetErrorString(e));
    }
// ... 16 lines not shown
```

include/tfbs_amd.h:

```cpp
#ifndef TFBS_AMD_H
#define TFBS_AMD_H

#include <stddef.h>
#include <stdint.h>

#ifdef __cplusplus
extern "C" {
#endif

#define TFBS_OK 0
#define TFBS_E_ARG (-1)
#define TFBS_E_BADBASE (-2)
#define TFBS_E_REFMISMATCH (-3)
#define TFBS_E_MNP (-4)
#define TFBS_E_PLOIDY (-5)
#define TFBS_E_RANGE (-6)
#define TFBS_E_PARSE (-7)
#define TFBS_E_IO (-8)
#define TFBS_E_HIP (-9)
#define TFBS_E_NODEVICE (-10)
#define TFBS_E_ALLELES (-11)
#define TFBS_E_ZEROLEN (-12)
#define TFBS_E_NOPATTERN (-13)
#define TFBS_E_STATE (-14)
// ... 80 lines not shown
int tfbs_ctx_scan_counters(tfbs_ctx *ctx, uint64_t out[5]);

int tfbs_matches(tfbs_ctx *ctx, const uint8_t *nucs, const uint64_t *pos, size_t n, uint32_t *counts,
                 uint64_t *out_start, uint64_t *out_end, size_t cap, size_t *n_total);

int tfbs_patch_haplotype(uint64_t range_start, uint64_t range_end, size_t n_diffs, const uint64_t *dpos,
                         const uint8_t *dref, const uint32_t *dnref, const uint8_t *dalt, const uint32_t *dnalt,
                         const uint8_t *ref_nucs, const uint64_t *ref_pos, size_t n_ref, uint8_t *out_nucs,
                         uint64_t *out_pos, size_t cap, size_t *n_out);

typedef struct tfbs_batch tfbs_batch;

int tfbs_batch_create(const tfbs_patterns *p, uint32_t n_samples, int keep_membership, tfbs_batch **out);
void tfbs_batch_destroy(tfbs_batch *b);
int tfbs_batch_add_bed(tfbs_batch *b, const char *basename);
int tfbs_batch_set_window_lmax(tfbs_batch *b, uint32_t lmax);
#define TFBS_GROUPER_HOST (-2)
int tfbs_batch_set_build_device(tfbs_batch *b, int device);
int tfbs_batch_hold(tfbs_batch *b, int on);
int tfbs_batch_build_stats(const tfbs_batch *b, uint64_t *dev_regions, uint64_t *host_regions);
int tfbs_batch_group_calls(const tfbs_batch *b, uint64_t *calls);
int tfbs_batch_patch_stats(const tfbs_batch *b, uint64_t *patched_regions);

typedef struct tfbs_grouper tfbs_grouper;
int tfbs_grouper_create(int device, tfbs_grouper **out);
void tfbs_grouper_destroy(tfbs_grouper *g);
int tfbs_grouper_group(tfbs_grouper *g, uint32_t H, size_t n_regions, const uint32_t *n_records,
                       const uint32_t *n_carriers, const uint32_t *ids, uint32_t *n_groups, uint64_t *masks,
                       uint32_t *counts, size_t cap, size_t *n_masks, uint16_t *rows);
int tfbs_batch_region_ext(const tfbs_batch *b, uint64_t merged_start, uint64_t merged_end, uint64_t *ext_start,
                          uint64_t *ext_end);
int tfbs_batch_region_begin(tfbs_batch *b, uint64_t merged_start, uint64_t merged_end, const char *ref_ascii,
                            size_t n_ref);
int tfbs_batch_region_add_inner(tfbs_batch *b, uint32_t bed, uint64_t start, uint64_t end);
int tfbs_batch_region_add_record_gt(tfbs_batch *b, uint64_t pos, uint32_t n_alleles, const char *ref,
                                    const char *alt, const int32_t *gt);
int tfbs_batch_region_add_record_carriers(tfbs_batch *b, uint64_t pos, const char *ref, const char *alt,
                                          const uint32_t *hap_ids, size_t n);
int tfbs_batch_region_end(tfbs_batch *b);

size_t tfbs_batch_num_regions(const tfbs_batch *b);
size_t tfbs_batch_num_haplotypes(const tfbs_batch *b);
uint64_t tfbs_batch_num_windows(const tfbs_batch *b);
uint64_t tfbs_batch_num_cell_ops(const tfbs_batch *b);
uint64_t tfbs_batch_num_effective_windows(const tfbs_batch *b);
uint64_t tfbs_batch_num_scan_windows(const tfbs_batch *b);
uint64_t tfbs_batch_num_scan_cell_ops(const tfbs_batch *b);
uint64_t tfbs_batch_input_bytes(const tfbs_batch *b);
uint64_t tfbs_batch_output_bytes(const tfbs_batch *b);

int tfbs_batch_upload(tfbs_ctx *ctx, tfbs_batch *b);
int tfbs_scan(tfbs_ctx *ctx, tfbs_batch *b);
int tfbs_batch_download(tfbs_ctx *ctx, tfbs_batch *b);
int tfbs_batch_reduce(tfbs_ctx *ctx, tfbs_batch *b);
int tfbs_batch_assemble(tfbs_ctx *ctx, tfbs_batch *b);
int tfbs_batch_assemble_wait(tfbs_ctx *ctx, tfbs_batch *b);
int tfbs_step(tfbs_ctx *ctx, tfbs_batch *b);
float tfbs_ctx_last_assemble_ms(const tfbs_ctx *ctx);
enum {
    TFBS_PATH_FAST = 1u << 0,
    TFBS_PATH_BIG = 1u << 1,
    TFBS_PATH_WALK = 1u << 2,
    TFBS_PATH_STEPBITS = 1u << 3,
    TFBS_PATH_DIRTY_LISTED = 1u << 4,
    TFBS_PATH_COR_ARENA = 1u << 5,
    TFBS_PATH_LISTS_SLICED = 1u << 6,
    TFBS_PATH_RUNS_L2 = 1u << 7,
    TFBS_PATH_HAP_GLOBAL = 1u << 8,
    TFBS_PATH_U32 = 1u << 9,
    TFBS_PATH_CNT_ARENA = 1u << 10,
    TFBS_PATH_TICKET = 1u << 11,
    TFBS_PATH_GIVEUP = 1u << 12,
    TFBS_PATH_WHY_SHIFT = 13,
    TFBS_PATH_ASM = 1u << 16,
    TFBS_PATH_ASM_HAPS = 1u << 17,
    TFBS_PATH_ASM_RUNS = 1u << 18,
    TFBS_PATH_ASM_HITS = 1u << 19,
    TFBS_PATH_ASM_REFS = 1u << 20,
    TFBS_PATH_ASM_SCRATCH = 1u << 21
};
#define TFBS_PATH_WHY(word) (((word) >> TFBS_PATH_WHY_SHIFT) & 7u)
int tfbs_ctx_assembly_trace(tfbs_ctx *ctx, int on);
int tfbs_batch_assembly_paths(tfbs_ctx *ctx, const tfbs_batch *b, uint32_t *mask, uint32_t n);
int tfbs_ctx_assembly_figures(tfbs_ctx *ctx, uint64_t out[8]);
int tfbs_ctx_post_figures(tfbs_ctx *ctx, uint64_t out[4]);
int tfbs_batch_region_layout(const tfbs_batch *b, size_t region, uint32_t out[4]);
int tfbs_batch_region_hap_runs(const tfbs_batch *b, size_t region, uint32_t h, int *reuses, uint32_t *run_off,
                               uint32_t *n_runs, uint32_t *ab, uint32_t cap);
int tfbs_batch_region_hap_own_runs(const tfbs_batch *b, size_t region, uint32_t h, int *reuses, uint32_t *run_off,
                                   uint32_t *n_runs, uint32_t *ab, uint32_t cap);
int tfbs_batch_encode(tfbs_ctx *ctx, tfbs_batch *b, size_t r0, size_t r1);
#define TFBS_ENC_DEVICE_CODES 1
int tfbs_batch_encode_flags(tfbs_ctx *ctx, tfbs_batch *b, size_t r0, size_t r1, int flags);
int tfbs_batch_encode_stats(const tfbs_batch *b, uint64_t out[7]);

int tfbs_batch_rows_bgzf(tfbs_ctx *ctx, tfbs_batch *b, size_t r0, size_t r1, const char *chromosome,
                         uint32_t min_maf, uint32_t *fake_position, int fd, uint64_t *bytes, uint64_t *n_rows,
                         uint64_t *text_bytes);
int tfbs_ctx_rows_bgzf_seconds(const tfbs_ctx *ctx, double *out);
int tfbs_ctx_rows_bgzf_blocks(const tfbs_ctx *ctx, uint64_t out[3]);

int tfbs_batch_region_num_keys(const tfbs_batch *b, size_t region, size_t *n);
int tfbs_batch_region_key(const tfbs_batch *b, size_t region, size_t k, uint32_t *bed, uint64_t *start,
                          uint64_t *end, uint16_t *pattern_id, uint32_t *left, uint32_t *right);
int tfbs_batch_rows(const tfbs_batch *b, const char *chromosome, uint32_t min_maf, uint32_t *fake_position,
                    char **text, size_t *len);
int tfbs_batch_region_rows(const tfbs_batch *b, size_t region, const char *chromosome, uint32_t min_maf,
                           uint32_t *fake_position, char **text, size_t *len);
int tfbs_batch_region_digest(const tfbs_batch *b, size_t region, uint64_t *digest);
int tfbs_batch_region_key_digest_sum(const tfbs_batch *b, size_t region, uint64_t *digest);
int tfbs_batch_region_input_digest(const tfbs_batch *b, size_t region, uint64_t *digest);
int tfbs_batch_region_digests(const tfbs_batch *b, size_t r0, size_t r1, uint32_t min_maf, uint32_t threads,
                              uint64_t *keys, uint64_t *rows, uint64_t *n_rows);
int tfbs_batch_region_stats(const tfbs_batch *b, size_t region, uint32_t *n_haplotypes, uint32_t *n_variants);
int tfbs_batch_format_rows(const tfbs_batch *b, const char *chromosome, uint32_t min_maf, uint32_t threads,
                           size_t r0, size_t r1, uint64_t *n_rows, uint64_t *n_bytes);
int tfbs_batch_prep_seconds(const tfbs_batch *b, double *out);
typedef struct tfbs_hit {
    uint32_t region, haplotype, pattern, window;
    uint64_t start, end;
    int32_t score;
    uint32_t reserved;
} tfbs_hit;

int tfbs_batch_hits(tfbs_ctx *ctx, tfbs_batch *b, size_t r0, size_t r1, tfbs_hit **out, size_t *n);
int tfbs_batch_hits_count(tfbs_ctx *ctx, tfbs_batch *b, size_t r0, size_t r1, uint64_t *per_region);
int tfbs_ctx_last_hits_ms(const tfbs_ctx *ctx, double out[4]);
int tfbs_batch_region_haplotype(const tfbs_batch *b, size_t region, uint32_t h, uint8_t *nucs, uint64_t *pos,
                                size_t cap, size_t *n, uint32_t *carriers);
int tfbs_batch_region_membership(const tfbs_batch *b, size_t region, uint32_t *out);
#define TFBS_HITS_ALL 0
#define TFBS_HITS_DIFF 1
#define TFBS_HITS_HEADER "#chrom\tregion\thaplotype\tcarriers\tkind\tname\tpattern_id\tstrand\tstart\tend\tscore\tcarrier_ids\n"
int tfbs_batch_hits_tsv(const tfbs_batch *b, const tfbs_hit *hits, size_t n, const char *chromosome, int mode,
                        char **text, size_t *len);

typedef struct tfbs_best {
    uint32_t region, haplotype, pattern, range;
    uint32_t window, n_windows;
    int32_t score;
    uint32_t reserved;
    uint64_t start, end;
} tfbs_best;

int tfbs_batch_best(tfbs_ctx *ctx, tfbs_batch *b, size_t r0, size_t r1, tfbs_best **out, size_t *n);
int tfbs_batch_region_num_ranges(const tfbs_batch *b, size_t region, size_t *n);
int tfbs_batch_region_range(const tfbs_batch *b, size_t region, size_t k, uint64_t *start, uint64_t *end);
int tfbs_ctx_last_best_ms(const tfbs_ctx *ctx, double out[2]);
#define TFBS_BEST_ALL 0
#define TFBS_BEST_DIFF 1
#define TFBS_BEST_HEADER "#chrom\tregion\tbed\tinner_start\tinner_end\tname\tpattern_id\thaplotype\tcarriers\tkind\tstrand\tstart\tend\tscore\tdelta\tcarrier_ids\n"
int tfbs_batch_best_tsv(const tfbs_batch *b, const tfbs_best *best, size_t n, const char *chromosome, int mode,
                        char **text, size_t *len);

uint64_t tfbs_affinity_weight(uint64_t d);
int tfbs_patterns_affinity_tops(const tfbs_patterns *p, int32_t *out);
typedef struct tfbs_affinity {
    uint32_t region, haplotype, pattern, range;
    uint32_t n_windows, n_nonzero;
    uint64_t sum;
} tfbs_affinity;
int tfbs_batch_affinity(tfbs_ctx *ctx, tfbs_batch *b, size_t r0, size_t r1, tfbs_affinity **out, size_t *n);
int tfbs_ctx_last_affinity_ms(const tfbs_ctx *ctx, double out[2]);
#define TFBS_AFFINITY_ALL 0
#define TFBS_AFFINITY_DIFF 1
#define TFBS_AFFINITY_HEADER "#chrom\tregion\tbed\tinner_start\tinner_end\tname\tpattern_id\thaplotype\tcarriers\tkind\ttop\tn_windows\taffinity\tdelta\tcarrier_ids\n"
// ... 149 lines not shown
```

Baseline: 312400 billion.

## Precompute per-region run ranges and hap reuse info in a separate kernel

Adds a region_asm kernel that runs once per upload/list build and precomputes, for each region, the min run offset, run count and max haplotype length, plus a per-haplotype packed reuse word. The key_fast assembly kernel reads these precomputed values instead of scanning DevHap records with shared-memory atomics and barriers at the start of each region. It also issues all front-end global loads (ref counts, ref hits, spill ranges, metadata, first runs, hitn) up front, using an asm barrier to overlap their latency. The aim is to shorten the serial prologue per region, at the cost of an extra kernel launch, memset and buffers. Profiling stamps are extended too.

After: 329800 billion (median of 6 runs). +5.5%, better.

```diff
diff --git a/find-tfbs_amd/__init__.py b/find-tfbs_amd/__init__.py
--- a/find-tfbs_amd/__init__.py
+++ b/find-tfbs_amd/__init__.py
@@ -360,6 +360,14 @@
 
     def assembly_trace(self, on=True):
         check(lib().tfbs_ctx_assembly_trace(self.h, 1 if on else 0))
+
+    def region_asm(self):
+        nr, nh = C.c_size_t(0), C.c_size_t(0)
+        check(lib().tfbs_ctx_region_asm(self.h, None, 0, None, 0, C.byref(nr), C.byref(nh)))
+        ra = (C.c_uint32 * (4 * max(nr.value, 1)))()
+        hr = (C.c_uint32 * max(nh.value, 1))()
+        check(lib().tfbs_ctx_region_asm(self.h, ra, max(nr.value, 1), hr, max(nh.value, 1), C.byref(nr), C.byref(nh)))
+        return ([tuple(ra[4 * r:4 * r + 4]) for r in range(nr.value)], list(hr[:nh.value]))
 
     def assembly_figures(self):
         out = (C.c_uint64 * 8)()
diff --git a/find-tfbs_amd/_capi.py b/find-tfbs_amd/_capi.py
--- a/find-tfbs_amd/_capi.py
+++ b/find-tfbs_amd/_capi.py
@@ -183,6 +183,8 @@
     ("tfbs_ctx_last_assemble_ms", C.c_float, [vp]),
     ("tfbs_ctx_assembly_trace", C.c_int, [vp, C.c_int]),
     ("tfbs_batch_assembly_paths", C.c_int, [vp, vp, u32p, C.c_uint32]),
+    ("tfbs_ctx_region_asm", C.c_int, [vp, u32p, C.c_size_t, u32p, C.c_size_t, C.POINTER(C.c_size_t),
+                                     C.POINTER(C.c_size_t)]),
     ("tfbs_ctx_assembly_figures", C.c_int, [vp, u64p]),
     ("tfbs_ctx_post_figures", C.c_int, [vp, u64p]),
     ("tfbs_batch_region_layout", C.c_int, [vp, C.c_size_t, u32p]),
diff --git a/find-tfbs_amd/csrc/ctx.hpp b/find-tfbs_amd/csrc/ctx.hpp
--- a/find-tfbs_amd/csrc/ctx.hpp
+++ b/find-tfbs_amd/csrc/ctx.hpp
@@ -81,6 +81,8 @@
     DevBuf<DevHap> haps;
     DevBuf<uint32_t> druns;
     DevBuf<DevRegion> regions;
+    DevBuf<uint32_t> hap_reuse;
+    DevBuf<uint4> region_asm;
     uint32_t n_regions = 0;
     const tfbs_batch *resident = nullptr;
     uint64_t upload_gen = 0;
@@ -88,6 +90,7 @@
     template <class F>
     void each_buf(F &&f) const {
         f(words), f(nmask), f(counts), f(posrel), f(inner), f(haps), f(druns), f(regions);
+        f(hap_reuse), f(region_asm);
     }
 };
 
diff --git a/find-tfbs_amd/csrc/ctx_assembly.hip b/find-tfbs_amd/csrc/ctx_assembly.hip
--- a/find-tfbs_amd/csrc/ctx_assembly.hip
+++ b/find-tfbs_amd/csrc/ctx_assembly.hip
@@ -7,6 +7,8 @@
     a.haps = ctx->img.haps.p;
     a.druns = ctx->img.druns.p;
     a.regions = ctx->img.regions.p;
+    a.hap_reuse = ctx->img.hap_reuse.p;
+    a.region_asm = ctx->img.region_asm.p;
     a.inner = ctx->img.inner.p;
     a.mmeta = ctx->tabs.m_meta.p;
     a.slot_mfma = ctx->tabs.slot_mfma.p;
@@ -110,8 +112,8 @@
         a.path = ctx->asmb.asm_path.p;
     }
     if (ctx->knobs.kf_prof_on && nr) {
-        if ((rc = ctx->asmb.kf_prof.ensure((size_t)nr * 16))) return rc;
-        HIP_TRY(hipMemsetAsync(ctx->asmb.kf_prof.p, 0, (size_t)nr * 128, ctx->stream));
+        if ((rc = ctx->asmb.kf_prof.ensure((size_t)nr * kKfProfWords))) return rc;
+        HIP_TRY(hipMemsetAsync(ctx->asmb.kf_prof.p, 0, (size_t)nr * kKfProfWords * 8, ctx->stream));
         a.prof = ctx->asmb.kf_prof.p;
     }
     if ((rc = launch_key_fast(a, nr, a.order ? ctx->asmb.asm_order_big : 0, ctx->stream, ctx->asmb.side, ctx->asmb.kf_fork,
@@ -129,29 +131,34 @@
 }
 
 static int kf_prof_report(tfbs_ctx *ctx, uint32_t nr) {
-    std::vector<uint64_t> h((size_t)nr * 16);
+    std::vector<uint64_t> h((size_t)nr * kKfProfWords);
     HIP_TRY(hipMemcpy(h.data(), ctx->asmb.kf_prof.p, h.size() * 8, hipMemcpyDeviceToHost));
     double ph[6] = {0, 0, 0, 0, 0, 0}, sz[8] = {0, 0, 0, 0, 0, 0, 0, 0}, mx = 0, at = 0;
+    double fr[5] = {0, 0, 0, 0, 0};
+    double tkt = 0;
     uint32_t n = 0;
     for (uint32_t r = 0; r < nr; r++) {
-        const uint64_t *p = &h[(size_t)r * 16];
+        const uint64_t *p = &h[(size_t)r * kKfProfWords];
         if (!p[6]) continue;
         n++;
         for (int k = 0; k < 6; k++) ph[k] += (double)(p[k + 1] - p[k]);
+        const uint64_t f[6] = {p[0], p[16], p[17], p[1], p[18], p[19]};
+        for (int k = 0; k < 5; k++) fr[k] += (double)(f[k + 1] - f[k]);
+        tkt += (double)p[20];
         mx = std::max(mx, (double)(p[6] - p[0]));
         at += (double)p[7];
         for (int k = 0; k < 8; k++) sz[k] += (double)p[8 + k];
     }
     std::vector<std::pair<double, uint32_t>> tot;
     for (uint32_t r = 0; r < nr; r++)
-        if (h[(size_t)r * 16 + 6]) tot.push_back({(double)(h[(size_t)r * 16 + 6] - h[(size_t)r * 16]), r});
+        if (h[(size_t)r * kKfProfWords + 6]) tot.push_back({(double)(h[(size_t)r * kKfProfWords + 6] - h[(size_t)r * kKfProfWords]), r});
     std::sort(tot.begin(), tot.end());
     if (!tot.empty()) {
         auto pct = [&](double f) { return tot[std::min(tot.size() - 1, (size_t)(f * tot.size()))].first; };
         fprintf(stderr, "[kf prof] total ticks p50 %.0f p90 %.0f p99 %.0f max %.0f; slowest regions (ticks U rows chunks "
                         "corrections refs):", pct(0.5), pct(0.9), pct(0.99), tot.back().first);
         for (size_t i = tot.size(); i-- > 0 && i + 6 > tot.size();) {
-            const uint64_t *p = &h[(size_t)tot[i].second * 16];
+            const uint64_t *p = &h[(size_t)tot[i].second * kKfProfWords];
             fprintf(stderr, " [%.0f %llu %llu %llu %llu %llu]", tot[i].first, (unsigned long long)p[8],
                     (unsigned long long)p[12], (unsigned long long)p[13], (unsigned long long)p[11],
                     (unsigned long long)p[15]);
@@ -161,7 +168,7 @@
     uint64_t t_lo = UINT64_MAX, t_hi = 0;
     double busy = 0;
     for (uint32_t r = 0; r < nr; r++) {
-        const uint64_t *p = &h[(size_t)r * 16];
+        const uint64_t *p = &h[(size_t)r * kKfProfWords];
         if (!p[6]) continue;
         t_lo = std::min(t_lo, p[0]);
         t_hi = std::max(t_hi, p[6]);
@@ -170,19 +177,19 @@
     {
         std::vector<std::pair<std::pair<uint64_t, uint64_t>, uint32_t>> ev;
         for (uint32_t r = 0; r < nr; r++)
-            if (h[(size_t)r * 16 + 6]) ev.push_back({{h[(size_t)r * 16 + 14], h[(size_t)r * 16]}, r});
+            if (h[(size_t)r * kKfProfWords + 6]) ev.push_back({{h[(size_t)r * kKfProfWords + 14], h[(size_t)r * kKfProfWords]}, r});
         std::sort(ev.begin(), ev.end());
         double gap = 0, late = 0, early_end = 0;
         uint32_t n_gap = 0, n_groups = 0;
         for (size_t i = 0; i < ev.size(); i++) {
-            const uint64_t *p = &h[(size_t)ev[i].second * 16];
+            const uint64_t *p = &h[(size_t)ev[i].second * kKfProfWords];
             const bool first = i == 0 || ev[i - 1].first.first != ev[i].first.first;
             const bool last = i + 1 == ev.size() || ev[i + 1].first.first != ev[i].first.first;
             if (first) {
                 n_groups++;
                 late += (double)(p[0] - t_lo);
             } else {
-                gap += (double)(p[0] - h[(size_t)ev[i - 1].second * 16 + 6]);
+                gap += (double)(p[0] - h[(size_t)ev[i - 1].second * kKfProfWords + 6]);
                 n_gap++;
             }
             if (last) early_end += (double)(t_hi - p[6]);
@@ -194,12 +201,17 @@
     }
     uint32_t early = 0;
     for (uint32_t r = 0; r < nr; r++)
-        if (h[(size_t)r * 16 + 6] && h[(size_t)r * 16] < t_lo + 1000) early++;
+        if (h[(size_t)r * kKfProfWords + 6] && h[(size_t)r * kKfProfWords] < t_lo + 1000) early++;
     if (t_hi > t_lo)
         fprintf(stderr, "[kf prof] span %.1f us (first region start to last end, 100 MHz ticks), region-time %.1f us: "
                         "%.0f regions in flight on average; %u regions started in the first 10 us\n",
                 (t_hi - t_lo) / 100.0, busy / 100.0, busy / (double)(t_hi - t_lo), early);
     const double d = n ? n : 1;
+    fprintf(stderr,
+            "[kf prof] front ticks/region: region record + reference hit list (round 1) %.0f, descriptors + hitn + "
+            "first runs + meta (round 2) %.0f, hitn scan %.0f, runs staged %.0f, reference hits + barrier %.0f; in front of "
+            "a region, ticket atomic to order entry %.0f\n",
+            fr[0] / d, fr[1] / d, fr[2] / d, fr[3] / d, fr[4] / d, tkt / d);
     fprintf(stderr,
             "[kf prof] regions %u of %u ticks/region: descr+hitn %.0f refs %.0f dirty %.0f lists %.0f keys %.0f "
             "chunks %.0f (of which var-list atomics %.0f) (max total %.0f); per region: U %.1f entries %.1f dirty-refs %.1f corrections %.1f rows "
diff --git a/find-tfbs_amd/csrc/ctx_scan.hip b/find-tfbs_amd/csrc/ctx_scan.hip
--- a/find-tfbs_amd/csrc/ctx_scan.hip
+++ b/find-tfbs_amd/csrc/ctx_scan.hip
@@ -28,6 +28,15 @@
     ctx->lists.wl_n_haps = n_haps;
     for (int c = 0; c < 2; c++) ctx->lists.sh_entries[c] = ctx->lists.sh_listed[c][0] = ctx->lists.sh_listed[c][1] = 0;
     if (B) B->lists_counted = false;
+    int rc;
+    {
+        const uint32_t nr = B ? (uint32_t)B->regions.size() : 1u;
+        if ((rc = ctx->img.hap_reuse.ensure(std::max<uint32_t>(n_haps, 1))) ||
+            (rc = ctx->img.region_asm.ensure(std::max<uint32_t>(nr, 1))) ||
+            (rc = launch_region_asm(ctx->img.haps.p, n_haps, ctx->img.regions.p, nr, ctx->img.hap_reuse.p,
+                                    ctx->img.region_asm.p, ctx->stream)))
+            return rc;
+    }
     if (P.m_supers.empty()) return TFBS_OK;
     const auto t0 = std::chrono::steady_clock::now();
     uint32_t lmin[2] = {0, 0}, span[2] = {0, 0};
@@ -36,7 +45,6 @@
         l = l ? std::min(l, S.lmin) : S.lmin;
         span[S.nk > 2 ? 1 : 0] = std::max(span[S.nk > 2 ? 1 : 0], S.lmax);
     }
-    int rc;
     for (int c = 0; c < 2; c++)
         if (lmin[c] && (rc = ctx->lists.wl_off[c].ensure((size_t)n_haps + 1))) return rc;
     if ((rc = ctx->lists.wl_tmp.ensure(scan_tmp_words((size_t)n_haps + 1))) ||
@@ -399,6 +407,21 @@
     return TFBS_OK;
 }
 
+int tfbs_ctx_region_asm(tfbs_ctx *ctx, uint32_t *region_asm, size_t cap_regions, uint32_t *hap_reuse, size_t cap_haps,
+                        size_t *n_regions, size_t *n_haps) {
+    if (!ctx || !n_regions || !n_haps || (cap_regions && !region_asm) || (cap_haps && !hap_reuse))
+        return tfbs::fail(TFBS_E_ARG, "bad argument");
+    *n_regions = ctx->img.n_regions;
+    *n_haps = ctx->lists.wl_n_haps;
+    if (!cap_regions && !cap_haps) return TFBS_OK;
+    if (*n_regions > cap_regions || *n_haps > cap_haps) return tfbs::fail(TFBS_E_ARG, "region asm: the arrays are too small");
+    HIP_TRY(hipSetDevice(ctx->device));
+    HIP_TRY(hipStreamSynchronize(ctx->stream));
+    if (*n_regions) HIP_TRY(hipMemcpy(region_asm, ctx->img.region_asm.p, *n_regions * 16, hipMemcpyDeviceToHost));
+    if (*n_haps) HIP_TRY(hipMemcpy(hap_reuse, ctx->img.hap_reuse.p, *n_haps * 4, hipMemcpyDeviceToHost));
+    return TFBS_OK;
+}
+
 int tfbs_batch_upload(tfbs_ctx *ctx, tfbs_batch *b) {
     if (!ctx || !b) return tfbs::fail(TFBS_E_ARG, "null argument");
     Batch &B = b->b;
diff --git a/find-tfbs_amd/csrc/key_kernels.hip b/find-tfbs_amd/csrc/key_kernels.hip
--- a/find-tfbs_amd/csrc/key_kernels.hip
+++ b/find-tfbs_amd/csrc/key_kernels.hip
@@ -50,6 +50,11 @@
     const uint32_t dk = (uint32_t)meta[kGDepth] - 1;
     const uint32_t key0 = (uint32_t)meta[kGStrandInts * sn + kGSlot] * rg.n_inner;
     return make_uint4(key0, i, L | (dk << 16), ref_overlaps(A, rg, L, i, 0, min(rg.n_inner, 32u)));
+}
+
+__device__ __forceinline__ uint4 make_ref_loaded(const AsmArgs &A, const DevRegion &rg, uint32_t L, uint32_t depth,
+                                                 uint32_t slot, uint32_t i) {
+    return make_uint4(slot * rg.n_inner, i, L | ((depth - 1) << 16), ref_overlaps(A, rg, L, i, 0, min(rg.n_inner, 32u)));
 }
 
 template <class F>
@@ -423,6 +428,8 @@
     *(__attribute__((address_space(1))) uint32_t *)p = v;
 }
 
+__device__ __forceinline__ void arrived(uint32_t &x) { asm volatile("" : "+v"(x)); }
+
 template <class Put>
 __device__ __forceinline__ void wave_push(Put &&put, uint32_t *n, uint32_t cap, bool want, uint32_t v) {
     const uint64_t m = __ballot(want);
@@ -479,15 +486,32 @@
     __shared__ uint32_t s_rkey[kFRows], s_rr[kFRows];
     __shared__ uint32_t s_loff[kFLists + 1], s_lidx[kFLists];
     __shared__ uint32_t s_w[kFWaves];
-    __shared__ uint32_t s_ncor, s_nref, s_run0, s_run1, s_nvar, s_arena, s_ndirty, s_lmax;
+    __shared__ uint32_t s_ncor, s_nref, s_nvar, s_arena, s_ndirty;
     __shared__ unsigned long long s_vbase, s_obase;
     const uint32_t tid = threadIdx.x, lane = tid & 63, wave = tid >> 6;
-    auto process = [&](const uint32_t r, const uint32_t by_ticket) {
+    auto process = [&](const uint32_t r, const uint32_t by_ticket, const uint64_t t_ticket) {
     auto stamp = [&](uint32_t k, uint64_t v) {
-        if (A.prof && tid == 0) A.prof[16 * (size_t)r + k] = v;
+        if (A.prof && tid == 0) A.prof[kKfProfWords * (size_t)r + k] = v;
     };
     stamp(0, wall_clock64());
-    const DevRegion rg = A.regions[r];
+    stamp(20, t_ticket);
+    uint32_t ft = tid;
+    arrived(ft);
+    const uint32_t *const none = reinterpret_cast<const uint32_t *>(A.regions + r);
+    auto have = [&](bool c, const auto *p) { return c ? p : reinterpret_cast<decltype(p)>(none); };
+    const bool spills = A.spill_count != nullptr;
+    uint32_t n_rc = ld_global(have(A.mfma, A.ref_count + r));
+    const uint2 rh = ld_global(have(A.mfma, reinterpret_cast<const uint2 *>(A.ref_hits) + (size_t)r * kRefPerRegion + (ft & 63u)));
+    uint32_t rh_g = rh.x, rh_i = rh.y;
+    uint32_t sp_n = ld_global(have(spills, A.spill_count));
+    uint32_t sp_c = ld_global(have(spills, A.spill_cnt + r));
+    uint32_t sp_o = ld_global(have(spills, A.spill_off + r));
+    DevRegion rg = A.regions[r];
+    uint4 ra = A.region_asm[r];
+    arrived(n_rc), arrived(rh_g), arrived(rh_i), arrived(sp_n), arrived(sp_c), arrived(sp_o);
+    arrived(rg.hap_count), arrived(ra.x);
+    if (!spills) sp_n = 0;
+    stamp(16, wall_clock64());
     const uint32_t U = rg.hap_count, n_inner = rg.n_inner, K = A.n_slots * n_inner;
     const uint64_t ko = (uint64_t)rg.inner_off * A.n_slots;
     uint32_t pw = TFBS_PATH_FAST | (kFBlock == 1024 ? TFBS_PATH_BIG : 0u) | by_ticket;
@@ -512,65 +536,59 @@
     if (U > (kFMaxU < A.fast_max_u ? kFMaxU : A.fast_max_u) || K > 32 * kFKeyWords || n_inner > 32) return give_up(0);
     const uint32_t hb = rg.hap_begin;
     const bool refs_on = A.mfma && rg.ref_hap != UINT32_MAX;
-    if (tid == 0) {
-        s_ncor = s_nref = s_run1 = s_ndirty = s_lmax = 0;
-        s_run0 = kFNone;
-    }
-    __syncthreads();
-    constexpr uint32_t kPer = kFMaxU / kFBlock;
-    uint32_t roff[kPer], rn[kPer], lmax = 0;
-#pragma unroll
-    for (uint32_t q = 0; q < kPer; q++) {
-        const uint32_t l = tid + q * kFBlock;
-        roff[q] = kFNone;
-        rn[q] = 0;
-        if (l < U) {
-            const DevHap &h = A.haps[hb + l];
-            lmax = max(lmax, h.len);
-            if (h.flags & HAP_DEDUP) {
-                roff[q] = h.rrun_off;
-                rn[q] = h.n_rruns;
-                atomicMin(&s_run0, h.rrun_off);
-                atomicMax(&s_run1, h.rrun_off + h.n_rruns);
-            }
-        }
-    }
+    const uint32_t run0 = (uint32_t)__builtin_amdgcn_readfirstlane((int)ra.x);
+    const uint32_t nruns = (uint32_t)__builtin_amdgcn_readfirstlane((int)ra.y);
+    const uint32_t lmax = (uint32_t)__builtin_amdgcn_readfirstlane((int)ra.z);
+    if (tid == 0) s_ncor = s_nref = s_ndirty = 0;
     const uint32_t g_lo = hb / A.hpb, g_hi = (hb + U - 1) / A.hpb;
     const uint32_t nl = A.mfma ? (g_hi + 1 - g_lo) * kMBlockWaves : 0u;
     auto list_idx = [&](uint32_t t) -> uint32_t { return g_lo * kMBlockWaves + t; };
-    uint32_t lcnt = 0, lidx = 0;
-    for (uint32_t t = tid; t < nl; t += kFBlock) {
-        const uint32_t i = list_idx(t);
-        if (t == tid) lidx = i;
-        lcnt += A.hitn[i];
+    const bool lists_staged = nl <= kFLists;
+    if (!lists_staged) pw |= TFBS_PATH_LISTS_SLICED;
+    if (nruns >= 65536) return give_up(2);
+    if (nruns > kFRuns) pw |= TFBS_PATH_RUNS_L2;
+    constexpr uint32_t kHapQ = kFHapLds / kFBlock;
+    uint32_t hx[kHapQ];
+#pragma unroll
+    for (uint32_t q = 0; q < kHapQ; q++) hx[q] = ld_global(A.hap_reuse + hb + min(ft + q * kFBlock, U - 1));
+    const uint32_t lidx = list_idx(min(ft, nl ? nl - 1 : 0u));
+    uint32_t lcnt = ld_global(have(nl != 0, A.hitn + lidx));
+    const bool runs_lds = nruns <= kFRuns;
+    const uint2 *const druns = reinterpret_cast<const uint2 *>(A.druns) + (nruns ? run0 : 0u);
+    const uint2 run_first = ld_global(have(runs_lds && nruns != 0, druns + min(ft, nruns ? nruns - 1 : 0u)));
+    uint32_t run_a = run_first.x, run_b = run_first.y;
+    const uint32_t n_list = refs_on ? min(n_rc, kRefPerRegion) : 0u;
+    const uint32_t g_ref = ft < n_list ? rh_g : 0u, sn = g_ref & 63u;
+    const uint32_t *const meta = have(refs_on, reinterpret_cast<const uint32_t *>(A.mmeta) + (size_t)(g_ref >> 6) * kGMetaInts);
+    uint32_t m_len = ld_global(meta + (refs_on ? kGStrandInts * sn + kGLen : 0u));
+    uint32_t m_depth = ld_global(meta + (refs_on ? (uint32_t)kGDepth : 0u));
+    uint32_t m_slot = ld_global(meta + (refs_on ? kGStrandInts * sn + kGSlot : 0u));
+#pragma unroll
+    for (uint32_t q = 0; q < kHapQ; q++) arrived(hx[q]);
+    arrived(lcnt), arrived(run_a), arrived(run_b), arrived(m_len), arrived(m_depth), arrived(m_slot);
+#pragma unroll
+    for (uint32_t q = 0; q < kHapQ; q++)
+        if (ft + q * kFBlock >= U) hx[q] = kFNone;
+    if (ft >= nl) lcnt = 0;
+    for (uint32_t t = ft + kFBlock; t < nl; t += kFBlock) lcnt += ld_global(A.hitn + list_idx(t));
+    stamp(17, wall_clock64());
+#pragma unroll
+    for (uint32_t q = 0; q < kHapQ; q++) {
+        const uint32_t l = tid + q * kFBlock;
+        if (l < U) s_hap[l] = hx[q];
     }
     uint32_t n_ent = 0;
     const uint32_t loff = block_excl_scan<kFWaves>(lcnt, s_w, n_ent);
-    if (tid == 0 && rg.ref_hap != UINT32_MAX) lmax = max(lmax, A.haps[rg.ref_hap].len);
-    if (lmax) atomicMax(&s_lmax, lmax);
-    const bool lists_staged = nl <= kFLists;
     if (lists_staged && tid < nl) {
         s_lidx[tid] = lidx;
         s_loff[tid] = loff;
     }
     if (lists_staged && tid == 0) s_loff[nl] = n_ent;
     stamp(1, wall_clock64());
-    const uint32_t run0 = s_run0, nruns = s_run0 == kFNone ? 0u : s_run1 - s_run0;
-    if (!lists_staged) pw |= TFBS_PATH_LISTS_SLICED;
-    if (nruns >= 65536) return give_up(2);
-    if (nruns > kFRuns) pw |= TFBS_PATH_RUNS_L2;
-#pragma unroll
-    for (uint32_t q = 0; q < kFHapLds / kFBlock; q++) {
-        const uint32_t l = tid + q * kFBlock;
-        if (l < U) s_hap[l] = roff[q] == kFNone ? kFNone : (roff[q] - run0) | (rn[q] << 16);
-    }
     auto hap_info = [&](uint32_t l) -> uint32_t {
         if (l < kFHapLds) return s_hap[l];
-        const DevHap &h = A.haps[hb + l];
-        return (h.flags & HAP_DEDUP) ? (h.rrun_off - run0) | (h.n_rruns << 16) : kFNone;
-    };
-    const bool runs_lds = nruns <= kFRuns;
-    const uint2 *const druns = reinterpret_cast<const uint2 *>(A.druns) + (nruns ? run0 : 0u);
+        return ld_global(A.hap_reuse + hb + l);
+    };
     auto run_at = [&](auto typed, uint32_t k) -> uint2 {
         if constexpr (decltype(typed)::value) {
             return s_run[k];
@@ -579,16 +597,16 @@
             return ld_global(druns + k);
         }
     };
-    if (runs_lds)
-        for (uint32_t k = tid; k < nruns; k += kFBlock)
-            s_run[k] = make_uint2(A.druns[2 * (run0 + k)], A.druns[2 * (run0 + k) + 1]);
-    const uint2 sp = spill_range(A, r);
+    if (runs_lds) {
+        if (tid < nruns) s_run[tid] = make_uint2(run_a, run_b);
+        for (uint32_t k = tid + kFBlock; k < nruns; k += kFBlock) s_run[k] = ld_global(druns + k);
+    }
+    stamp(18, wall_clock64());
+    const uint2 sp = sp_n && sp_c ? make_uint2(sp_o, sp_o + sp_c) : make_uint2(0, 0);
     if (refs_on) {
-        const uint32_t n = min(A.ref_count[r], kRefPerRegion);
-        if (tid < n) {
-            const size_t o = 2 * ((size_t)r * kRefPerRegion + tid);
+        if (tid < n_list) {
             const uint32_t at = atomicAdd(&s_nref, 1u);
-            if (at < kFRefs) s_ref[at] = make_ref(A, rg, A.ref_hits[o], A.ref_hits[o + 1]);
+            if (at < kFRefs) s_ref[at] = make_ref_loaded(A, rg, m_len, m_depth, m_slot, rh_i);
         }
         for (uint32_t e = sp.x + tid; e < sp.y; e += kFBlock) {
             const uint32_t *q = A.spill_sorted + 3 * (size_t)e;
@@ -600,6 +618,7 @@
     }
     __syncthreads();
     const uint32_t nref = s_nref;
+    stamp(19, wall_clock64());
     if (nref > kFRefs) return give_up(3);
     const bool pairwise = (uint64_t)U * nref <= 65536;
     if (!pairwise) pw |= TFBS_PATH_WALK;
@@ -861,7 +880,7 @@
     else lists_and_rows(KfAny{});
     stamp(5, wall_clock64());
     auto row_of = [&](uint32_t j) { return s_rbase[j >> 5] + __popc(s_bits[j >> 5] & ((1u << (j & 31)) - 1u)); };
-    const bool half = 4 * (s_lmax + 64) < 65536 && A.cor_lds != 0;
+    const bool half = 4 * (lmax + 64) < 65536 && A.cor_lds != 0;
     uint32_t rows_per = min((half ? 2 : 1) * kFCnt / U, kFRows);
     uint16_t *const cnt16 = reinterpret_cast<uint16_t *>(s_cnt);
     bool h16 = half, cnt_arena = false;
@@ -1011,8 +1030,14 @@
     uint32_t i = blockIdx.x;
     while (i < count) {
         uint32_t tk = 0;
+        uint64_t t_ticket = A.prof ? wall_clock64() : 0;
         if (tickets && tid == 0) tk = gridDim.x + atomicAdd(A.next + which, 1u);
-        process(A.order ? A.order[first + i] : first + i, i == blockIdx.x ? 0u : (uint32_t)TFBS_PATH_TICKET);
+        const uint32_t r = A.order ? A.order[first + i] : first + i;
+        if (A.prof) {
+            asm volatile("" ::"v"(r));
+            t_ticket = wall_clock64() - t_ticket;
+        }
+        process(r, i == blockIdx.x ? 0u : (uint32_t)TFBS_PATH_TICKET, t_ticket);
         if (!tickets) break;
         if (tid == 0) s_tk = tk;
         __syncthreads();
diff --git a/find-tfbs_amd/csrc/keys.hpp b/find-tfbs_amd/csrc/keys.hpp
--- a/find-tfbs_amd/csrc/keys.hpp
+++ b/find-tfbs_amd/csrc/keys.hpp
@@ -15,6 +15,8 @@
     const DevHap *haps;
     const uint32_t *druns;
     const DevRegion *regions;
+    const uint32_t *hap_reuse;
+    const uint4 *region_asm;
     const int32_t *inner;
     const int32_t *mmeta;
     const uint8_t *slot_mfma;
@@ -57,6 +59,8 @@
     uint32_t grid_cap;
 };
 
+constexpr uint32_t kKfProfWords = 24;
+
 enum AsmCtr : uint32_t {
     kCtrOver = 0,
     kCtrRedoN = 2,
diff --git a/find-tfbs_amd/csrc/scan.hpp b/find-tfbs_amd/csrc/scan.hpp
--- a/find-tfbs_amd/csrc/scan.hpp
+++ b/find-tfbs_amd/csrc/scan.hpp
@@ -124,6 +124,8 @@
                        const uint32_t *words = nullptr, const ClassTab *tab = nullptr,
                        int (*ensure_share)(void *ctx, int c, uint64_t n, uint2 **p) = nullptr,
                        uint64_t shared[2] = nullptr, uint64_t listed[2][2] = nullptr);
+int launch_region_asm(const DevHap *haps, uint32_t n_haps, const DevRegion *regions, uint32_t n_regions,
+                      uint32_t *hap_reuse, uint4 *region_asm, hipStream_t stream);
 size_t mfma_lds_fixed();
 
 }
diff --git a/find-tfbs_amd/csrc/window_lists.hip b/find-tfbs_amd/csrc/window_lists.hip
--- a/find-tfbs_amd/csrc/window_lists.hip
+++ b/find-tfbs_amd/csrc/window_lists.hip
@@ -249,6 +249,36 @@
     }
 }
 
+__global__ __launch_bounds__(256) void region_asm_kernel(const DevHap *__restrict__ haps,
+                                                          const DevRegion *__restrict__ regions, uint32_t n_regions,
+                                                          uint32_t *__restrict__ hap_reuse, uint4 *__restrict__ region_asm) {
+    const uint32_t lane = threadIdx.x & 63;
+    for (uint32_t r = blockIdx.x * 4 + (threadIdx.x >> 6); r < n_regions; r += gridDim.x * 4) {
+        const DevRegion rg = regions[r];
+        uint32_t lo = UINT32_MAX, hi = 0, lmax = 0;
+        for (uint32_t l = lane; l < rg.hap_count; l += 64) {
+            const DevHap &h = haps[rg.hap_begin + l];
+            lmax = max(lmax, h.len);
+            if (h.flags & HAP_DEDUP) {
+                lo = min(lo, h.rrun_off);
+                hi = max(hi, h.rrun_off + h.n_rruns);
+            }
+        }
+        if (lane == 0 && rg.ref_hap != UINT32_MAX) lmax = max(lmax, haps[rg.ref_hap].len);
+#pragma unroll
+        for (int o = 32; o; o >>= 1) {
+            lo = min(lo, (uint32_t)__shfl_xor((int)lo, o));
+            hi = max(hi, (uint32_t)__shfl_xor((int)hi, o));
+            lmax = max(lmax, (uint32_t)__shfl_xor((int)lmax, o));
+        }
+        for (uint32_t l = lane; l < rg.hap_count; l += 64) {
+            const DevHap &h = haps[rg.hap_begin + l];
+            hap_reuse[rg.hap_begin + l] = (h.flags & HAP_DEDUP) ? (h.rrun_off - lo) | (h.n_rruns << 16) : UINT32_MAX;
+        }
+        if (lane == 0) region_asm[r] = make_uint4(lo, lo == UINT32_MAX ? 0u : hi - lo, lmax, 0u);
+    }
+}
+
 constexpr uint32_t kScanThreads = 1024, kScanTile = 4 * kScanThreads;
 __global__ __launch_bounds__(kScanThreads) void scan_tile_kernel(uint64_t *__restrict__ x, uint64_t n,
                                                                  uint64_t *__restrict__ sums) {
@@ -297,6 +327,18 @@
     }
     const hipError_t e = hipGetLastError();
     if (e != hipSuccess) return fail(TFBS_E_HIP, std::string("scan kernels: ") + hipGetErrorString(e));
+    return TFBS_OK;
+}
+
+int launch_region_asm(const DevHap *haps, uint32_t n_haps, const DevRegion *regions, uint32_t n_regions,
+                      uint32_t *hap_reuse, uint4 *region_asm, hipStream_t stream) {
+    hipError_t e = hipMemsetAsync(hap_reuse, 0xFF, (size_t)std::max<uint32_t>(n_haps, 1) * 4, stream);
+    if (e == hipSuccess && n_regions) {
+        hipLaunchKernelGGL(region_asm_kernel, dim3(std::min<uint32_t>((n_regions + 3) / 4, 2048)), dim3(256), 0, stream, haps,
+                           regions, n_regions, hap_reuse, region_asm);
+        e = hipGetLastError();
+    }
+    if (e != hipSuccess) return fail(TFBS_E_HIP, std::string("region_asm_kernel: ") + hipGetErrorString(e));
     return TFBS_OK;
 }
 
diff --git a/include/tfbs_amd.h b/include/tfbs_amd.h
--- a/include/tfbs_amd.h
+++ b/include/tfbs_amd.h
@@ -186,6 +186,8 @@
 #define TFBS_PATH_WHY(word) (((word) >> TFBS_PATH_WHY_SHIFT) & 7u)
 int tfbs_ctx_assembly_trace(tfbs_ctx *ctx, int on);
 int tfbs_batch_assembly_paths(tfbs_ctx *ctx, const tfbs_batch *b, uint32_t *mask, uint32_t n);
+int tfbs_ctx_region_asm(tfbs_ctx *ctx, uint32_t *region_asm, size_t cap_regions, uint32_t *hap_reuse, size_t cap_haps,
+                        size_t *n_regions, size_t *n_haps);
 int tfbs_ctx_assembly_figures(tfbs_ctx *ctx, uint64_t out[8]);
 int tfbs_ctx_post_figures(tfbs_ctx *ctx, uint64_t out[4]);
 int tfbs_batch_region_layout(const tfbs_batch *b, size_t region, uint32_t out[4]);
```
